# alibaba/TorchEasyRec

Hardware: NVIDIA H100
Metric: samples/sec (DLRM-Criteo synth, train step fwd+bwd+optimizer) (higher is better)
Workload: dtype f32

## Files before the change

include/tzk.h:

```cpp
#ifndef TZK_H_
#define TZK_H_

#include <stddef.h>
#include <stdint.h>

#ifdef __cplusplus
extern "C" {
#endif

#define TZK_ABI_VERSION 1

#define TZK_POOL_SUM 0
#define TZK_POOL_MEAN 1

#define TZK_OPT_SGD 0
#define TZK_OPT_ADAGRAD 1
#define TZK_OPT_ROWWISE_ADAGRAD 2
#define TZK_OPT_ADAM 3
#define TZK_OPT_PARTIAL_ROWWISE_ADAM 4
#define TZK_OPT_LAMB 5
#define TZK_OPT_PARTIAL_ROWWISE_LAMB 6
#define TZK_OPT_LARS_SGD 7
#define TZK_OPT_ACCUM_OUT 100

// ... 53 lines not shown
                                   const int64_t* offsets, const float* per_sample_weights, int32_t F, int32_t B,
                                   int32_t max_dim, int32_t vec_ok, float* out, int64_t ld_out, tzk_stream_t stream);

size_t tzk_fused_bwd_workspace_bytes(int64_t nnz, int64_t total_keys, int32_t max_dim);
int tzk_fused_bwd(int32_t optimizer, int32_t pooled, const float* grad_out, int64_t ld_grad,
                  const int64_t* feat_w_off, const int64_t* feat_rows, const int32_t* feat_dim,
                  const int32_t* feat_col, const int32_t* feat_pool, const int64_t* feat_key_base,
                  const int64_t* ids, const int64_t* offsets, int32_t F, int32_t B, int64_t nnz,
                  int64_t total_keys, int32_t max_dim, int32_t vec_ok, float* weights, float* state,
                  float lr, float eps, float grad_scale, void* workspace, size_t workspace_bytes,
                  tzk_stream_t stream);
int tzk_fused_bwd_ex(const tzk_opt_args* opt, int32_t pooled, const float* grad_out, int64_t ld_grad,
                     const int64_t* feat_w_off, const int64_t* feat_rows, const int32_t* feat_dim,
                     const int32_t* feat_col, const int32_t* feat_pool, const int64_t* feat_key_base,
                     const int64_t* ids, const int64_t* offsets, int32_t F, int32_t B, int64_t nnz,
                     int64_t total_keys, int32_t max_dim, int32_t vec_ok, float* weights, float grad_scale,
                     void* workspace, size_t workspace_bytes, tzk_stream_t stream);
int tzk_fused_bwd_apply_ex(const tzk_opt_args* opt, int32_t pooled, const float* grad_out, int64_t ld_grad,
                           const int64_t* feat_w_off, const int64_t* feat_rows, const int32_t* feat_dim,
                           const int32_t* feat_col, const int32_t* feat_pool, const int64_t* feat_key_base,
                           const int64_t* offsets, int32_t F, int32_t B, int64_t nnz, int64_t total_keys,
                           int32_t max_dim, int32_t vec_ok, float* weights, float grad_scale, void* workspace,
                           size_t workspace_bytes, tzk_stream_t stream);
int tzk_fused_bwd_sort(int32_t pooled, const int64_t* feat_rows, const int64_t* feat_key_base, const int64_t* ids,
                       const int64_t* offsets, int32_t F, int32_t B, int64_t nnz, int64_t total_keys,
                       int32_t max_dim, void* workspace, size_t workspace_bytes, tzk_stream_t stream);
int tzk_fused_bwd_apply(int32_t optimizer, int32_t pooled, const float* grad_out, int64_t ld_grad,
                        const int64_t* feat_w_off, const int64_t* feat_rows, const int32_t* feat_dim,
                        const int32_t* feat_col, const int32_t* feat_pool, const int64_t* feat_key_base,
                        const int64_t* offsets, int32_t F, int32_t B, int64_t nnz, int64_t total_keys,
                        int32_t max_dim, int32_t vec_ok, float* weights, float* state, float lr, float eps,
                        float grad_scale, void* workspace, size_t workspace_bytes, tzk_stream_t stream);

size_t tzk_fused_bwd_weighted_workspace_bytes(int64_t nnz, int64_t total_keys, int32_t max_dim);
int tzk_fused_bwd_sort_weighted(int32_t pooled, const int64_t* feat_rows, const int64_t* feat_key_base, const int64_t* ids,
                                const int64_t* offsets, const float* per_sample_weights, int32_t F, int32_t B,
                                int64_t nnz, int64_t total_keys, int32_t max_dim, void* workspace,
                                size_t workspace_bytes, tzk_stream_t stream);

int tzk_bag_grad_expand(const float* grad_out, int64_t ld_grad, const int32_t* feat_col,
                        const int32_t* feat_pool, const int64_t* offsets, const int32_t* slot, int32_t F,
                        int32_t B, int32_t D, float* g_rows, tzk_stream_t stream);

size_t tzk_bucketize_rw_workspace_bytes(int32_t F, int32_t B, int32_t W, int64_t nnz);
int tzk_bucketize_rw(const int64_t* ids, const int64_t* offsets, int32_t F, int32_t B, int32_t W,
                     const int64_t* feat_block, const int32_t* feat_owner, int64_t nnz,
                     int64_t wire_capacity, int32_t* out_lengths, int64_t* out_offsets, int64_t* out_ids,
                     int32_t* out_pos, int32_t* out_inv, void* workspace, size_t workspace_bytes,
                     tzk_stream_t stream);

int tzk_permute_lengths(const int32_t* lengths, const int32_t* perm, int32_t S_out, int32_t B,
                        int32_t* out_lengths, tzk_stream_t stream);
int tzk_permute_ids(const int64_t* ids, const int64_t* in_offsets, const int64_t* out_offsets,
                    const int32_t* perm, int32_t S_out, int32_t B, int64_t* out_ids,
                    tzk_stream_t stream);
int tzk_permute_weights(const float* weights, const int64_t* in_offsets, const int64_t* out_offsets,
                        const int32_t* perm, int32_t S_out, int32_t B, float* out_weights, tzk_stream_t stream);

int tzk_col_gather_sum(const float* const* srcs_host, const int64_t* src_ld_host, int32_t n_src,
                       const int32_t* col_start, const int32_t* col_src, const int32_t* col_srccol,
                       int32_t C, int64_t rows, float* out, int64_t ld_out, tzk_stream_t stream);

int tzk_jagged_to_padded(const float* values, const int64_t* offsets, int32_t B, int32_t T, int32_t D,
                         float* out, tzk_stream_t stream);
int tzk_padded_to_jagged(const float* grad_out, const int64_t* offsets, int32_t B, int32_t T, int32_t D,
                         int64_t nnz, float* grad_values, tzk_stream_t stream);

int tzk_fm_fwd(const float* x, int64_t ld_x, int64_t B, int32_t N, int32_t D, float* y, int64_t ld_y,
               tzk_stream_t stream);
int tzk_fm_bwd(const float* x, int64_t ld_x, const float* dy, int64_t ld_dy, int64_t B, int32_t N,
               int32_t D, float* dx, int64_t ld_dx, tzk_stream_t stream);

int tzk_dot_interact_fwd(const float* dense, int64_t ld_dense, const float* sparse, int64_t ld_sparse,
                         int64_t B, int32_t Ns, int32_t D, int32_t copy_dense, int32_t copy_sparse,
                         int32_t p_pad, float* out, int64_t ld_out, tzk_stream_t stream);
int tzk_dot_interact_bwd(const float* dense, int64_t ld_dense, const float* sparse, int64_t ld_sparse,
                         const float* d_out, int64_t ld_dout, int64_t B, int32_t Ns, int32_t D,
                         int32_t copy_dense, int32_t copy_sparse, int32_t p_pad, float* d_dense,
                         int64_t ld_ddense, float* d_sparse, int64_t ld_dsparse, tzk_stream_t stream);
int tzk_interact_wide_bwd(const float* dz, int64_t ld_dz, const float* w, int64_t ld_w, const float* dense,
                          int64_t ld_dense, const float* sparse, int64_t ld_sparse, int64_t M, float* d_dense,
                          int64_t ld_ddense, float* d_sparse, int64_t ld_dsparse, float* wt_hi, float* wt_lo,
                          tzk_stream_t stream);
int tzk_interact_wide_fwd(const float* dense, int64_t ld_dense, const float* sparse, int64_t ld_sparse, const float* w,
                          int64_t ld_w, const float* bias, int64_t M, float* y, int64_t ld_y, float* pairs,
                          int64_t ld_pairs, float* w_hi, float* w_lo, tzk_stream_t stream);
int tzk_interact_wide_wgrad(const float* dz, int64_t ld_dz, const float* pairs, int64_t ld_pairs, const float* dense,
                            int64_t ld_dense, const float* sparse, int64_t ld_sparse, int64_t M, int32_t slabs,
                            float* partial, float* dw, int64_t ld_dw, tzk_stream_t stream);

int tzk_bias_act(float* y, int64_t ld_y, const float* bias, int64_t M, int32_t N, int32_t relu,
                 tzk_stream_t stream);
size_t tzk_act_bwd_colsum_workspace_bytes(int64_t M, int32_t N);
int tzk_act_bwd_colsum(const float* dy, int64_t ld_dy, const float* y, int64_t ld_y, int64_t M, int32_t N,
                       int32_t relu, float* dz, int64_t ld_dz, float* colsum, void* workspace,
                       size_t workspace_bytes, tzk_stream_t stream);

int tzk_small_linear_fwd(const float* x, int64_t ld_x, const float* w, const float* bias, int64_t M, int32_t K,
                         int32_t N, int32_t relu, float* y, int64_t ld_y, tzk_stream_t stream);
size_t tzk_small_linear_bwd_workspace_bytes(int64_t M, int32_t K, int32_t N);
int tzk_small_linear_bwd(const float* x, int64_t ld_x, const float* w, const float* y, int64_t ld_y,
                         const float* dy, int64_t ld_dy, int64_t M, int32_t K, int32_t N, int32_t relu, float* dx,
                         int64_t ld_dx, float* dw, float* db, void* workspace, size_t workspace_bytes,
                         tzk_stream_t stream);
size_t tzk_bce_logits_workspace_bytes(int64_t M);

size_t tzk_tower_tail_bce_workspace_bytes(int64_t M, int32_t K, int32_t N);
int tzk_tower_tail_bce(const float* y1, int64_t ld_y, const float* w1, const float* b1, const float* w2, const float* b2,
                       const float* labels, int64_t M, int32_t K, int32_t N, float* logits, float* dy1, int64_t ld_dy,
                       float* out, void* workspace, size_t workspace_bytes, tzk_stream_t stream);
int tzk_bce_logits_fwd_bwd(const float* logits, const float* labels, int64_t M, float* loss, float* dlogits,
                           void* workspace, size_t workspace_bytes, tzk_stream_t stream);

int tzk_din_attn_input_fwd(const float* query, int64_t ld_q, int32_t Dq, const float* seq, const int64_t* offsets,
                           int32_t B, int32_t Ds, int64_t N, float* out, tzk_stream_t stream);
int tzk_din_attn_input_bwd(const float* d_in, const float* query, int64_t ld_q, int32_t Dq, const float* seq,
                           const int64_t* offsets, int32_t B, int32_t Ds, int64_t N, float* d_query, float* d_seq,
                           tzk_stream_t stream);
int tzk_jagged_softmax_wsum_fwd(const float* scores, const float* seq, const int64_t* offsets, int32_t B, int32_t Ds,
                                int32_t max_len, int64_t N, float* probs, float* out, tzk_stream_t stream);
int tzk_jagged_softmax_wsum_bwd(const float* d_out, const float* probs, const float* seq, const int64_t* offsets,
                                int32_t B, int32_t Ds, int32_t max_len, int64_t N, float* d_scores, float* d_seq,
                                tzk_stream_t stream);

int tzk_peer_pooled_gather_fwd(const uint64_t* table_ptrs, const int64_t* rf_w_off, const int64_t* feat_rows,
                               const int64_t* feat_block, const int32_t* feat_owner, const int32_t* feat_dim,
                               const int32_t* feat_col, const int32_t* feat_pool, const int64_t* ids,
                               const int64_t* offsets, int32_t F, int32_t B, int32_t W, int32_t max_dim, float* out,
                               int64_t ld_out, const float* mirror, const int64_t* feat_mirror_off, tzk_stream_t stream);
int tzk_peer_pooled_gather_fwd_sel(const uint64_t* table_ptrs, const int64_t* rf_w_off, const int64_t* feat_rows,
                                   const int64_t* feat_block, const int32_t* feat_owner, const int32_t* feat_dim,
                                   const int32_t* feat_col, const int32_t* feat_pool, const int64_t* ids,
                                   const int64_t* offsets, int32_t F, int32_t B, int32_t W, int32_t max_dim, float* out,
                                   int64_t ld_out, const float* mirror, const int64_t* feat_mirror_off,
                                   const int32_t* feat_sel, int32_t n_sel, tzk_stream_t stream);
int tzk_peer_seq_gather_fwd(const uint64_t* table_ptrs, const int64_t* rf_w_off, const int64_t* feat_rows,
                            const int64_t* feat_block, const int32_t* feat_owner, const int64_t* ids,
                            const int64_t* offsets, int32_t F, int32_t B, int32_t W, int32_t D, int64_t nnz, float* out,
                            const float* mirror, const int64_t* feat_mirror_off, tzk_stream_t stream);
int tzk_peer_mirror_refresh(const uint64_t* table_ptrs, int32_t W, const int32_t* seg_rank, const int64_t* seg_src,
                            const int64_t* seg_dst, const int64_t* seg_n, int32_t n_seg, float* mirror,
                            tzk_stream_t stream);
int tzk_peer_barrier(const uint64_t* pad_ptrs, int32_t me, int32_t W, uint32_t* epoch, tzk_stream_t stream);
size_t tzk_peer_bucketize_workspace_bytes(int32_t F, int32_t B, int32_t W);
int tzk_peer_bucketize(const int64_t* ids, const int64_t* offsets, int32_t F, int32_t B, int32_t W,
                       const int64_t* feat_block, const int32_t* feat_owner, const int64_t* feat_rows,
                       const int64_t* rf_key_base, int32_t pooled, int64_t cap, int64_t* wire_key, int32_t* wire_idx,
                       int32_t* counts, void* workspace, size_t workspace_bytes, tzk_stream_t stream);
int tzk_peer_publish_grad(const float* grad, int64_t ld_grad, const int32_t* feat_col, const int32_t* feat_dim,
                          const int32_t* feat_pool, const int64_t* offsets, int32_t F, int32_t B, float* dst,
                          int64_t ld_dst, tzk_stream_t stream);
int tzk_peer_push_grad(const uint64_t* recv_ptrs, const float* grad, int64_t ld_grad, const int32_t* feat_col,
                       const int32_t* feat_pool, const int64_t* offsets, const int32_t* wire_idx, const int32_t* counts,
                       int32_t me, int32_t W, int64_t cap, int32_t B, int32_t D, int32_t pooled, tzk_stream_t stream);
int tzk_peer_allreduce_mean(const uint64_t* src_ptrs, int32_t W, int64_t n, float* out, tzk_stream_t stream);
int tzk_peer_small_update(const tzk_opt_args* opt, const uint64_t* psum_ptrs, const uint64_t* flag_ptrs, int32_t W,
                          const void* tabs, int32_t n_tabs, int32_t total_rows, int32_t max_dim, float* weights,
                          tzk_stream_t stream);
int tzk_fused_bwd_sort_peer(const uint64_t* key_ptrs, const uint64_t* idx_ptrs, const uint64_t* count_ptrs, int32_t me,
                            int32_t W, int64_t cap, int32_t idx_span, int64_t total_keys, int32_t max_dim,
                            int32_t* overflow, void* workspace, size_t workspace_bytes, tzk_stream_t stream);
int tzk_fused_bwd_apply_peer(const tzk_opt_args* opt, int32_t pooled, const uint64_t* grad_ptrs, int64_t ld_grad,
                             const int64_t* feat_w_off, const int64_t* feat_rows, const int32_t* feat_dim,
                             const int32_t* feat_col, const int32_t* feat_pool, const int64_t* feat_key_base, int32_t F,
                             int32_t B, int32_t me, int32_t W, int64_t cap, int32_t idx_span, int64_t total_keys,
                             int32_t max_dim, int32_t vec_ok, float* weights, float grad_scale, void* workspace,
                             size_t workspace_bytes, tzk_stream_t stream);

int tzk_peer_pooled_gather_fwd_weighted(const uint64_t* table_ptrs, const int64_t* rf_w_off, const int64_t* feat_rows,
                                        const int64_t* feat_block, const int32_t* feat_owner, const int32_t* feat_dim,
                                        const int32_t* feat_col, const int32_t* feat_pool, const int64_t* ids,
                                        const int64_t* offsets, int32_t F, int32_t B, int32_t W, int32_t max_dim,
                                        float* out, int64_t ld_out, const float* mirror, const int64_t* feat_mirror_off,
                                        const float* per_sample_weights, const int32_t* feat_sel, int32_t n_sel,
                                        tzk_stream_t stream);
int tzk_peer_bucketize_weighted(const int64_t* ids, const int64_t* offsets, int32_t F, int32_t B, int32_t W,
                                const int64_t* feat_block, const int32_t* feat_owner, const int64_t* feat_rows,
                                const int64_t* rf_key_base, int32_t pooled, int64_t cap, int64_t* wire_key,
                                int32_t* wire_idx, int32_t* counts, void* workspace, size_t workspace_bytes,
                                const float* per_sample_weights, float* wire_w, tzk_stream_t stream);
int tzk_peer_push_grad_weighted(const uint64_t* recv_ptrs, const float* grad, int64_t ld_grad, const int32_t* feat_col,
                                const int32_t* feat_pool, const int64_t* offsets, const int32_t* wire_idx,
                                const int32_t* counts, int32_t me, int32_t W, int64_t cap, int32_t B, int32_t D,
                                int32_t pooled, const float* wire_w, tzk_stream_t stream);

int tzk_dot_interact27_fwd_bf16(const uint16_t* dense, int64_t ld_dense, const float* sparse, int64_t ld_sparse, int64_t B,
                                uint16_t* out, int64_t ld_out, tzk_stream_t stream);
int tzk_dot_interact27_bwd_bf16(const uint16_t* d_out, int64_t ld_dout, const uint16_t* dense, int64_t ld_dense,
                                const float* sparse, int64_t ld_sparse, int64_t B, uint16_t* d_dense, int64_t ld_ddense,
                                float* d_sparse, int64_t ld_dsparse, tzk_stream_t stream);

int tzk_binned_auc_update(const void* preds, int32_t pred_dtype, const void* labels, int32_t label_dtype, int64_t n,
                          const float* thresholds, int32_t T, int64_t* counts, int64_t* invalid, tzk_stream_t stream);
// ... 145 lines not shown
```

torcheasyrec_b200/_lib.py:

```python

import ctypes
import os
from ctypes import c_char_p, c_float, c_int32, c_int64, c_size_t, c_void_p

_HERE = os.path.dirname(os.path.abspath(__file__))
LIB_PATH = os.path.join(_HERE, "csrc", "libtzk.so")

P = c_void_p

class TzkOptArgs(ctypes.Structure):

    _fields_ = [("optimizer", c_int32), ("lr", c_float), ("eps", c_float), ("beta1", c_float), ("beta2", c_float),
                ("weight_decay", c_float), ("max_gradient", c_float), ("state", c_void_p), ("state2", c_void_p),
                ("step", c_void_p), ("weights_f16", c_int32), ("interleaved", c_int32), ("momentum", c_float),
                ("eta", c_float), ("weight_decay_mode", c_int32), ("per_sample_weights", c_void_p)]


PLE_MAX_GATES, PLE_MAX_EXPERTS, PLE_MAX_GATE_EXPERTS = 9, 64, 32


class TzkPleGateArgs(ctypes.Structure):

    _fields_ = [("B", c_int64), ("H", c_int32), ("n_experts", c_int32), ("n_inputs", c_int32), ("n_gates", c_int32),
                ("in_dim", c_int32 * PLE_MAX_GATES), ("gate_input", c_int32 * PLE_MAX_GATES),
# ... 46 lines not shown
    "tzk_sm_count": (c_int32, []),
    "tzk_lengths_to_offsets_workspace_bytes": (c_size_t, [c_int64]),
    "tzk_lengths_to_offsets": (c_int32, [P, c_int64, P, P, c_size_t, P]),
    "tzk_pooled_gather_fwd": (
        c_int32,
        [P, P, P, P, P, P, P, P, c_int32, c_int32, c_int32, c_int32, P, c_int64, P],
    ),
    "tzk_seq_gather_fwd": (c_int32, [P, P, P, P, P, c_int32, c_int32, c_int32, c_int64, P, P]),
    "tzk_pooled_gather_fwd_f16": (
        c_int32,
        [P, P, P, P, P, P, P, P, c_int32, c_int32, c_int32, c_int32, P, c_int64, P],
    ),
    "tzk_seq_gather_fwd_f16": (c_int32, [P, P, P, P, P, c_int32, c_int32, c_int32, c_int64, P, P]),
    "tzk_pooled_gather_fwd_strided": (
        c_int32,
        [P, P, P, P, P, P, P, P, P, c_int32, c_int32, c_int32, c_int32, P, c_int64, P],
    ),
    "tzk_seq_gather_fwd_strided": (c_int32, [P, P, P, P, P, c_int32, c_int32, c_int32, c_int32, c_int64, P, P]),
    "tzk_pooled_gather_fwd_weighted": (
        c_int32,
        [P, c_int32, P, P, P, P, P, P, P, P, P, c_int32, c_int32, c_int32, c_int32, P, c_int64, P],
    ),
    "tzk_fused_bwd_workspace_bytes": (c_size_t, [c_int64, c_int64, c_int32]),
    "tzk_fused_bwd_weighted_workspace_bytes": (c_size_t, [c_int64, c_int64, c_int32]),
    "tzk_fused_bwd_sort_weighted": (
        c_int32, [c_int32, P, P, P, P, P, c_int32, c_int32, c_int64, c_int64, c_int32, P, c_size_t, P]),
    "tzk_fused_bwd": (
        c_int32,
        [c_int32, c_int32, P, c_int64, P, P, P, P, P, P, P, P, c_int32, c_int32, c_int64, c_int64, c_int32,
         c_int32, P, P, c_float, c_float, c_float, P, c_size_t, P],
    ),
    "tzk_fused_bwd_ex": (
        c_int32,
        [P, c_int32, P, c_int64, P, P, P, P, P, P, P, P, c_int32, c_int32, c_int64, c_int64, c_int32, c_int32, P,
         c_float, P, c_size_t, P],
    ),
    "tzk_fused_bwd_apply_ex": (
        c_int32,
        [P, c_int32, P, c_int64, P, P, P, P, P, P, P, c_int32, c_int32, c_int64, c_int64, c_int32, c_int32, P,
         c_float, P, c_size_t, P],
    ),
    "tzk_fused_bwd_sort": (c_int32, [c_int32, P, P, P, P, c_int32, c_int32, c_int64, c_int64, c_int32, P, c_size_t, P]),
    "tzk_fused_bwd_apply": (
        c_int32,
        [c_int32, c_int32, P, c_int64, P, P, P, P, P, P, P, c_int32, c_int32, c_int64, c_int64, c_int32,
         c_int32, P, P, c_float, c_float, c_float, P, c_size_t, P],
    ),
    "tzk_bucketize_rw_workspace_bytes": (c_size_t, [c_int32, c_int32, c_int32, c_int64]),
    "tzk_bucketize_rw": (
        c_int32,
        [P, P, c_int32, c_int32, c_int32, P, P, c_int64, c_int64, P, P, P, P, P, P, c_size_t, P],
    ),
    "tzk_bag_grad_expand": (c_int32, [P, c_int64, P, P, P, P, c_int32, c_int32, c_int32, P, P]),
    "tzk_permute_lengths": (c_int32, [P, P, c_int32, c_int32, P, P]),
    "tzk_permute_ids": (c_int32, [P, P, P, P, c_int32, c_int32, P, P]),
    "tzk_permute_weights": (c_int32, [P, P, P, P, c_int32, c_int32, P, P]),
    "tzk_col_gather_sum": (c_int32, [P, P, c_int32, P, P, P, c_int32, c_int64, P, c_int64, P]),
    "tzk_jagged_to_padded": (c_int32, [P, P, c_int32, c_int32, c_int32, P, P]),
    "tzk_padded_to_jagged": (c_int32, [P, P, c_int32, c_int32, c_int32, c_int64, P, P]),
    "tzk_fm_fwd": (c_int32, [P, c_int64, c_int64, c_int32, c_int32, P, c_int64, P]),
    "tzk_fm_bwd": (c_int32, [P, c_int64, P, c_int64, c_int64, c_int32, c_int32, P, c_int64, P]),
    "tzk_dot_interact_fwd": (
        c_int32,
        [P, c_int64, P, c_int64, c_int64, c_int32, c_int32, c_int32, c_int32, c_int32, P, c_int64, P],
    ),
    "tzk_bias_act": (c_int32, [P, c_int64, P, c_int64, c_int32, c_int32, P]),
    "tzk_act_bwd_colsum_workspace_bytes": (c_size_t, [c_int64, c_int32]),
    "tzk_act_bwd_colsum": (c_int32, [P, c_int64, P, c_int64, c_int64, c_int32, c_int32, P, c_int64, P, P, c_size_t, P]),
    "tzk_small_linear_fwd": (c_int32, [P, c_int64, P, P, c_int64, c_int32, c_int32, c_int32, P, c_int64, P]),
    "tzk_small_linear_bwd_workspace_bytes": (c_size_t, [c_int64, c_int32, c_int32]),
    "tzk_small_linear_bwd": (
        c_int32,
        [P, c_int64, P, P, c_int64, P, c_int64, c_int64, c_int32, c_int32, c_int32, P, c_int64, P, P, P, c_size_t, P],
    ),
    "tzk_bce_logits_workspace_bytes": (c_size_t, [c_int64]),
    "tzk_bce_logits_fwd_bwd": (c_int32, [P, P, c_int64, P, P, P, c_size_t, P]),
    "tzk_dot_interact_bwd": (
        c_int32,
        [P, c_int64, P, c_int64, P, c_int64, c_int64, c_int32, c_int32, c_int32, c_int32, c_int32, P, c_int64, P,
         c_int64, P],
    ),
    "tzk_interact_wide_bwd": (
        c_int32, [P, c_int64, P, c_int64, P, c_int64, P, c_int64, c_int64, P, c_int64, P, c_int64, P, P, P]),
    "tzk_interact_wide_fwd": (
        c_int32, [P, c_int64, P, c_int64, P, c_int64, P, c_int64, P, c_int64, P, c_int64, P, P, P]),
    "tzk_interact_wide_wgrad": (
        c_int32, [P, c_int64, P, c_int64, P, c_int64, P, c_int64, c_int64, c_int32, P, P, c_int64, P]),
    "tzk_tower_tail_bce_workspace_bytes": (c_size_t, [c_int64, c_int32, c_int32]),
    "tzk_tower_tail_bce": (c_int32, [P, c_int64, P, P, P, P, P, c_int64, c_int32, c_int32, P, P, c_int64, P, P, c_size_t, P]),
    "tzk_din_attn_input_fwd": (c_int32, [P, c_int64, c_int32, P, P, c_int32, c_int32, c_int64, P, P]),
    "tzk_din_attn_input_bwd": (c_int32, [P, P, c_int64, c_int32, P, P, c_int32, c_int32, c_int64, P, P, P]),
    "tzk_jagged_softmax_wsum_fwd": (c_int32, [P, P, P, c_int32, c_int32, c_int32, c_int64, P, P, P]),
    "tzk_jagged_softmax_wsum_bwd": (c_int32, [P, P, P, P, c_int32, c_int32, c_int32, c_int64, P, P, P]),
    "tzk_peer_pooled_gather_fwd": (
        c_int32, [P, P, P, P, P, P, P, P, P, P, c_int32, c_int32, c_int32, c_int32, P, c_int64, P, P, P]),
    "tzk_peer_pooled_gather_fwd_sel": (
        c_int32, [P, P, P, P, P, P, P, P, P, P, c_int32, c_int32, c_int32, c_int32, P, c_int64, P, P, P, c_int32, P]),
    "tzk_peer_seq_gather_fwd": (
        c_int32, [P, P, P, P, P, P, P, c_int32, c_int32, c_int32, c_int32, c_int64, P, P, P, P]),
    "tzk_peer_mirror_refresh": (c_int32, [P, c_int32, P, P, P, P, c_int32, P, P]),
    "tzk_peer_barrier": (c_int32, [P, c_int32, c_int32, P, P]),
    "tzk_peer_bucketize_workspace_bytes": (c_size_t, [c_int32, c_int32, c_int32]),
    "tzk_peer_bucketize": (
        c_int32, [P, P, c_int32, c_int32, c_int32, P, P, P, P, c_int32, c_int64, P, P, P, P, c_size_t, P]),
    "tzk_peer_publish_grad": (c_int32, [P, c_int64, P, P, P, P, c_int32, c_int32, P, c_int64, P]),
    "tzk_peer_push_grad": (
        c_int32, [P, P, c_int64, P, P, P, P, P, c_int32, c_int32, c_int64, c_int32, c_int32, c_int32, P]),
    "tzk_peer_allreduce_mean": (c_int32, [P, c_int32, c_int64, P, P]),
    "tzk_peer_small_update": (c_int32, [P, P, P, c_int32, P, c_int32, c_int32, c_int32, P, P]),
    "tzk_fused_bwd_sort_peer": (
        c_int32, [P, P, P, c_int32, c_int32, c_int64, c_int32, c_int64, c_int32, P, P, c_size_t, P]),
    "tzk_fused_bwd_apply_peer": (
        c_int32,
        [P, c_int32, P, c_int64, P, P, P, P, P, P, c_int32, c_int32, c_int32, c_int32, c_int64, c_int32, c_int64,
         c_int32, c_int32, P, c_float, P, c_size_t, P]),
    "tzk_peer_pooled_gather_fwd_weighted": (
        c_int32, [P, P, P, P, P, P, P, P, P, P, c_int32, c_int32, c_int32, c_int32, P, c_int64, P, P, P, P, c_int32, P]),
    "tzk_peer_bucketize_weighted": (
        c_int32, [P, P, c_int32, c_int32, c_int32, P, P, P, P, c_int32, c_int64, P, P, P, P, c_size_t, P, P, P]),
    "tzk_peer_push_grad_weighted": (
        c_int32, [P, P, c_int64, P, P, P, P, P, c_int32, c_int32, c_int64, c_int32, c_int32, c_int32, P, P]),
    "tzk_dot_interact27_fwd_bf16": (c_int32, [P, c_int64, P, c_int64, c_int64, P, c_int64, P]),
    "tzk_dot_interact27_bwd_bf16": (
        c_int32, [P, c_int64, P, c_int64, P, c_int64, c_int64, P, c_int64, P, c_int64, P]),
    "tzk_binned_auc_update": (c_int32, [P, c_int32, P, c_int32, c_int64, P, c_int32, P, P, P]),
    "tzk_peer_pooled_gather_fwd_f16": (
        c_int32, [P, P, P, P, P, P, P, P, P, P, c_int32, c_int32, c_int32, c_int32, P, c_int64, P, P, P]),
    "tzk_peer_pooled_gather_fwd_sel_f16": (
        c_int32, [P, P, P, P, P, P, P, P, P, P, c_int32, c_int32, c_int32, c_int32, P, c_int64, P, P, P, c_int32, P]),
    "tzk_peer_pooled_gather_fwd_weighted_f16": (
        c_int32, [P, P, P, P, P, P, P, P, P, P, c_int32, c_int32, c_int32, c_int32, P, c_int64, P, P, P, P, c_int32, P]),
    "tzk_peer_seq_gather_fwd_f16": (
        c_int32, [P, P, P, P, P, P, P, c_int32, c_int32, c_int32, c_int32, c_int64, P, P, P, P]),
    "tzk_peer_mirror_refresh_f16": (c_int32, [P, c_int32, P, P, P, P, c_int32, P, P]),
    "tzk_wukong_mix_fwd": (
        c_int32, [P, P, P, P, P, P, c_int64, c_int32, c_int32, c_int32, c_int32, c_int32, c_int32, P, P, P, P]),
    "tzk_wukong_mix_bwd": (
        c_int32,
        [P, P, P, P, P, P, P, P, c_int64, c_int32, c_int32, c_int32, c_int32, c_int32, c_int32, P, P, P, P]),
    "tzk_wukong_out_fwd": (c_int32, [P, P, P, P, c_int64, c_int32, c_int32, c_int32, c_int32, P, P, P]),
    "tzk_wukong_out_bwd": (
        c_int32, [P, P, P, P, P, c_int64, c_int32, c_int32, c_int32, c_int32, P, P, P, P, P]),
    "tzk_masknet_mask_fwd": (c_int32, [P, c_int32, P, P, P, P, c_int64, c_int32, c_int32, c_int32, P, P, P]),
    "tzk_masknet_mask_bwd": (
        c_int32, [P, c_int32, P, P, P, P, P, P, c_int64, c_int32, c_int32, c_int32, P, P, P, P, P]),
    "tzk_masknet_ffn_fwd": (c_int32, [P, P, P, P, c_int64, c_int32, c_int32, c_int32, P, P, P]),
    "tzk_masknet_ffn_bwd": (c_int32, [P, P, P, P, P, P, c_int64, c_int32, c_int32, c_int32, P, P, P, P]),
    "tzk_ple_gate_smem_bytes": (c_int64, [P, c_int32]),
    "tzk_ple_gate_fwd": (c_int32, [P, c_int32, P, P, P]),
    "tzk_ple_gate_bwd": (c_int32, [P, P, P, c_int32, P, P, P, P]),
    "tzk_pepnet_gate_fwd": (c_int32, [P, c_int32, P]),
    "tzk_pepnet_gate_bwd": (c_int32, [P, c_int32, P, P, P]),
    "tzk_jrc_loss_workspace_bytes": (c_size_t, [c_int64]),
    "tzk_jrc_loss": (c_int32, [P, c_int64, P, P, P, c_int64, c_float, c_int32, P, P, P, c_size_t, P]),
    "tzk_rocket_head_fwd": (c_int32, [P, c_int32, P, P, P]),
    "tzk_rocket_head_bwd": (c_int32, [P, P, P, c_int32, P, P, P]),
}

_lib = None


class TzkError(RuntimeError):
    pass


def lib() -> ctypes.CDLL:
    global _lib
    if _lib is None:
        if not os.path.exists(LIB_PATH):
            raise TzkError(
                f"{LIB_PATH} not found: build it with `python -m torcheasyrec_b200.csrc.build` "
                "(or __graft_entry__.build()).  There is no CPU fallback."
# ... 17 lines not shown
```

torcheasyrec_b200/csrc/tzk_common.cuh:

```cuda
#pragma once
#include <stdlib.h>
#include <cuda_fp16.h>
#include <cuda_runtime.h>
#include <stdint.h>
#include <stdio.h>

#include "../../include/tzk.h"

namespace tzk {

void set_error(const char* fmt, ...);

inline cudaStream_t as_stream(tzk_stream_t s) { return reinterpret_cast<cudaStream_t>(s); }

#define TZK_CHECK_LAUNCH(name)                                                      \
  do {                                                                              \
    cudaError_t e__ = cudaGetLastError();                                           \
    if (e__ != cudaSuccess) {                                                       \
      ::tzk::set_error("%s: launch failed: %s", name, cudaGetErrorString(e__));     \
      return 2;                                                                     \
    }                                                                               \
  } while (0)

#define TZK_REQUIRE(cond, ...)        \
  do {                                \
    if (!(cond)) {                    \
      ::tzk::set_error(__VA_ARGS__);  \
      return 1;                       \
    }                                 \
  } while (0)

constexpr int kSmCountH100 = 132;

inline bool unvalidated_switch(const char* name) {
  const char* e = getenv(name);
  if (e && (e[0] == '0' || e[0] == '1')) return e[0] == '1';
  const char* x = getenv("TZK_EXPERIMENTAL");
  return x && x[0] == '1';
}

__host__ __device__ inline int64_t ceil_div64(int64_t a, int64_t b) { return (a + b - 1) / b; }
inline size_t align_up(size_t x, size_t a) { return (x + a - 1) / a * a; }
__host__ __device__ inline size_t align16(size_t x) { return (x + 15) / 16 * 16; }

__device__ __forceinline__ float4 ld_row_f4(const float* p) {
  float4 r;
  asm("ld.global.nc.L1::no_allocate.v4.f32 {%0,%1,%2,%3}, [%4];"
               : "=f"(r.x), "=f"(r.y), "=f"(r.z), "=f"(r.w)
               : "l"(p));
  return r;
}
__device__ __forceinline__ float4 ld_coh_f4(const float* p) {
  float4 r;
  asm("ld.global.L1::no_allocate.v4.f32 {%0,%1,%2,%3}, [%4];" : "=f"(r.x), "=f"(r.y), "=f"(r.z), "=f"(r.w) : "l"(p));
  return r;
}
__device__ __forceinline__ float4 ld_rw_f4(const float* p) {
  float4 r;
  asm volatile("ld.global.L1::no_allocate.v4.f32 {%0,%1,%2,%3}, [%4];"
               : "=f"(r.x), "=f"(r.y), "=f"(r.z), "=f"(r.w)
               : "l"(p)
               : "memory");
  return r;
}
__device__ __forceinline__ float4 ld_row_h4(const __half* p) {
  unsigned int a, b;
  asm("ld.global.nc.L1::no_allocate.v2.u32 {%0,%1}, [%2];" : "=r"(a), "=r"(b) : "l"(p));
  const float2 lo = __half22float2(*reinterpret_cast<const __half2*>(&a));
  const float2 hi = __half22float2(*reinterpret_cast<const __half2*>(&b));
  return make_float4(lo.x, lo.y, hi.x, hi.y);
}
template <typename WT> __device__ __forceinline__ float4 ld_table_f4(const WT* p);
template <> __device__ __forceinline__ float4 ld_table_f4<float>(const float* p) { return ld_row_f4(p); }
template <> __device__ __forceinline__ float4 ld_table_f4<__half>(const __half* p) { return ld_row_h4(p); }
template <typename WT> __device__ __forceinline__ float ld_table_f1(const WT* p);
template <> __device__ __forceinline__ float ld_table_f1<float>(const float* p) { return __ldg(p); }
template <> __device__ __forceinline__ float ld_table_f1<__half>(const __half* p) { return __half2float(__ldg(p)); }

__device__ __forceinline__ void st_stream_f4(float* p, const float4& v) {
  asm volatile("st.global.L1::no_allocate.v4.f32 [%0], {%1,%2,%3,%4};" ::"l"(p), "f"(v.x), "f"(v.y),
               "f"(v.z), "f"(v.w)
               : "memory");
}
__device__ __forceinline__ float4 f4_add(const float4& a, const float4& b) {
  return make_float4(a.x + b.x, a.y + b.y, a.z + b.z, a.w + b.w);
}
__device__ __forceinline__ float4 f4_scale(const float4& a, float s) {
  return make_float4(a.x * s, a.y * s, a.z * s, a.w * s);
}

}
```

torcheasyrec_b200/csrc/tzk_dense.cu:

```cuda
#include <cstdlib>

#include "tzk_common.cuh"

using namespace tzk;

#include "tzk_launch.cuh"
namespace tzk_itc {
__device__ __forceinline__ uint32_t cvt_tf32(float x) {
  uint32_t r;
  asm("cvt.rna.tf32.f32 %0, %1;" : "=r"(r) : "f"(x));
  return r;
}
__device__ __forceinline__ void mma_tf32(float (&c)[4], const uint32_t (&a)[4], const uint32_t (&b)[2]) {
  asm volatile("mma.sync.aligned.m16n8k8.row.col.f32.tf32.tf32.f32 {%0,%1,%2,%3}, {%4,%5,%6,%7}, {%8,%9}, {%0,%1,%2,%3};"
               : "+f"(c[0]), "+f"(c[1]), "+f"(c[2]), "+f"(c[3])
               : "r"(a[0]), "r"(a[1]), "r"(a[2]), "r"(a[3]), "r"(b[0]), "r"(b[1]));
}
}
#include "tzk_interact_tc.cuh"


namespace {
constexpr int kThreads = 256;

// ... 657 lines not shown
  const int64_t stride = (int64_t)gridDim.x * blockDim.x;
  for (int64_t i = (int64_t)blockIdx.x * blockDim.x + threadIdx.x; i < n; i += stride) {
    const int64_t r = i / N;
    const int c = (int)(i - r * N);
    float v = y[r * ld + c] + (bias ? __ldg(bias + c) : 0.f);
    if (relu) v = v > 0.f ? v : 0.f;
    y[r * ld + c] = v;
  }
}

__global__ void __launch_bounds__(kThreads)
bias_act_vec_kernel(float* __restrict__ y, int64_t ld, const float* __restrict__ bias, int n4_total, int N4,
                    int relu) {
  const int stride = gridDim.x * blockDim.x;
  for (int i = blockIdx.x * blockDim.x + threadIdx.x; i < n4_total; i += stride) {
    const int r = i / N4, c4 = i - r * N4;
    float4* p = reinterpret_cast<float4*>(y + (int64_t)r * ld) + c4;
    float4 v = *p;
    if (bias) {
      const float4 b = __ldg(reinterpret_cast<const float4*>(bias) + c4);
      v.x += b.x; v.y += b.y; v.z += b.z; v.w += b.w;
    }
    if (relu) {
      v.x = v.x > 0.f ? v.x : 0.f; v.y = v.y > 0.f ? v.y : 0.f;
      v.z = v.z > 0.f ? v.z : 0.f; v.w = v.w > 0.f ? v.w : 0.f;
    }
    *p = v;
  }
}

constexpr int kSlabRows = 128;
__global__ void __launch_bounds__(kThreads)
act_bwd_colsum_kernel(const float* __restrict__ dy, int64_t ld_dy, const float* __restrict__ y, int64_t ld_y,
                      int64_t M, int N, int relu, float* __restrict__ dz, int64_t ld_dz,
                      float* __restrict__ partial) {
  __shared__ float red[kThreads];
  const int rg = kThreads / N;
  const int c = threadIdx.x % N, r0 = threadIdx.x / N;
  const int64_t row_lo = (int64_t)blockIdx.x * kSlabRows;
  const int64_t row_hi = row_lo + kSlabRows < M ? row_lo + kSlabRows : M;
  float acc = 0.f;
#pragma unroll 4
  for (int64_t r = row_lo + r0; r < row_hi; r += rg) {
    float g = __ldg(dy + r * ld_dy + c);
    if (relu && !(__ldg(y + r * ld_y + c) > 0.f)) g = 0.f;
    if (dz) dz[r * ld_dz + c] = g;
    acc += g;
  }
  red[threadIdx.x] = acc;
  __syncthreads();
  if (r0 == 0) {
    float s = 0.f;
    for (int k = 0; k < rg; ++k) s += red[k * N + c];
    partial[(int64_t)blockIdx.x * N + c] = s;
  }
}

__global__ void __launch_bounds__(256)
colsum_final_kernel(const float* __restrict__ partial, int64_t n_blocks, int N, float* __restrict__ out) {
  __shared__ float red[8][32];
  const int o = threadIdx.x & 31, g = threadIdx.x >> 5;
  const int c = blockIdx.x * 32 + o;
  float s = 0.f;
  if (c < N) {
    int64_t b = g;
    for (; b + 24 < n_blocks; b += 32) {
      const float a0 = partial[b * N + c], a1 = partial[(b + 8) * N + c];
      const float a2 = partial[(b + 16) * N + c], a3 = partial[(b + 24) * N + c];
      s += a0; s += a1; s += a2; s += a3;
    }
    for (; b < n_blocks; b += 8) s += partial[b * N + c];
  }
  red[g][o] = s;
  __syncthreads();
  if (g == 0 && c < N) {
    float r = 0.f;
#pragma unroll
    for (int k = 0; k < 8; ++k) r += red[k][o];
    out[c] = r;
  }
}
}

extern "C" int tzk_bias_act(float* y, int64_t ld_y, const float* bias, int64_t M, int32_t N, int32_t relu,
                            tzk_stream_t stream) {
  TZK_REQUIRE(M >= 0 && N >= 1, "bias_act: bad sizes");
  if (M == 0) return 0;
  TZK_REQUIRE(y != nullptr, "bias_act: y is NULL");
  const bool vec = (N % 4 == 0) && (ld_y % 4 == 0) && ((uintptr_t)y % 16 == 0) &&
                   (!bias || (uintptr_t)bias % 16 == 0) && (M * N / 4 < ((int64_t)1 << 31));
  if (vec)
    bias_act_vec_kernel<<<grid_for(M * N / 4, kThreads, kSmCountH100 * 16), kThreads, 0, as_stream(stream)>>>(
        y, ld_y, bias, (int)(M * N / 4), N / 4, relu);
  else
    bias_act_kernel<<<grid_for(M * N, kThreads, kSmCountH100 * 16), kThreads, 0, as_stream(stream)>>>(y, ld_y, bias,
                                                                                                    M, N, relu);
  TZK_CHECK_LAUNCH("bias_act_kernel");
  return 0;
}

extern "C" size_t tzk_act_bwd_colsum_workspace_bytes(int64_t M, int32_t N) {
  return (size_t)ceil_div64(M < 1 ? 1 : M, kSlabRows) * (size_t)(N < 1 ? 1 : N) * sizeof(float);
}

extern "C" int tzk_act_bwd_colsum(const float* dy, int64_t ld_dy, const float* y, int64_t ld_y, int64_t M,
                                  int32_t N, int32_t relu, float* dz, int64_t ld_dz, float* colsum,
                                  void* workspace, size_t workspace_bytes, tzk_stream_t stream) {
  TZK_REQUIRE(M >= 1 && N >= 1, "act_bwd_colsum: bad sizes");
  TZK_REQUIRE(N <= kThreads && kThreads % N == 0, "act_bwd_colsum: N=%d must divide %d", N, kThreads);
  TZK_REQUIRE(dy && colsum && (!relu || y), "act_bwd_colsum: NULL argument");
  TZK_REQUIRE(workspace && workspace_bytes >= tzk_act_bwd_colsum_workspace_bytes(M, N),
              "act_bwd_colsum: workspace too small");
  const int64_t nb = ceil_div64(M, kSlabRows);
  float* partial = static_cast<float*>(workspace);
  act_bwd_colsum_kernel<<<(unsigned)nb, kThreads, 0, as_stream(stream)>>>(dy, ld_dy, y, ld_y, M, N, relu, dz, ld_dz,
                                                                          partial);
  TZK_CHECK_LAUNCH("act_bwd_colsum_kernel");
  colsum_final_kernel<<<(N + 31) / 32, 256, 0, as_stream(stream)>>>(partial, nb, N, colsum);
  TZK_CHECK_LAUNCH("colsum_final_kernel");
  return 0;
}
```

torcheasyrec_b200/csrc/tzk_interact_wide.cu:

```cuda
#include <stdint.h>
#include <stdio.h>
#include <stdlib.h>

#ifdef TZK_CPU_SHIM
#include "cuda_cpu_shim.h"
#include "sm90_cpu_emu.h"
#include "sm90_wgmma_emu.h"
typedef void* tzk_stream_t;
inline void mbar_arrive(uint64_t* bar) { mbar_expect_tx(bar, 0); }
#define TZK_REQUIRE(cond, ...) do { if (!(cond)) return 1; } while (0)
#define TZK_CHECK_LAUNCH(name) do {} while (0)
#else
#include <cuda.h>
#include "tzk_common.cuh"
#define TZK_DYN_SMEM(type, name) extern __shared__ __align__(1024) type name[]
#include "tzk_launch.cuh"
#endif

namespace {
#ifndef TZK_CPU_SHIM
#include "tzk_sm90_ptx.h"
#endif
#include "tzk_tma.h"
#include "tzk_wgmma.cuh"
namespace tzk_itc {
__device__ __forceinline__ uint32_t cvt_tf32(float x) { return tf32_bits(x); }
__device__ __forceinline__ void mma_tf32(float (&c)[4], const uint32_t (&a)[4], const uint32_t (&b)[2]) { ::mma_tf32(c, a, b); }
}
#include "tzk_interact_tc.cuh"

__device__ __forceinline__ float4 load_l2(const float* p) {
#ifdef TZK_CPU_SHIM
  return *reinterpret_cast<const float4*>(p);
#else
  return __ldcg(reinterpret_cast<const float4*>(p));
#endif
}

constexpr int FB_M = 64;
constexpr int FB_THREADS = 512;
constexpr int FB_WARPS = FB_THREADS / 32;
constexpr int FB_CHUNKS = (tzk_itc::kRow + 31) / 32;
constexpr int FB_PAIR_CHUNKS = tzk_itc::kInter / 32;
constexpr int FB_ITEMS = 1 + FB_CHUNKS;
constexpr int FB_BOX = 32 * 128;
constexpr int FB_HALF = 2 * FB_BOX;
constexpr int FB_STAGE = 2 * FB_HALF;
constexpr int FB_STAGES = 4;
constexpr int FB_LDP = 360;
constexpr int FB_P_OFF = FB_STAGES * FB_STAGE;
constexpr int FB_S_OFF = FB_P_OFF + FB_M * FB_LDP * 4;
constexpr int FB_IJ_OFF = FB_S_OFF + FB_WARPS * 32 * tzk_itc::kSS * 4;
constexpr int FB_BAR_OFF = FB_IJ_OFF + tzk_itc::kInter * 2;
constexpr int FB_SMEM = FB_BAR_OFF + 4 * FB_STAGES * 8;
static_assert(FB_HALF == FB_M * 128, "a dZ box [64 x 32 floats] fills half a stage");
static_assert(FB_STAGES == 4, "stage i % 4 is read by warpgroup i % 4");
static_assert(FB_SMEM <= 227 * 1024, "over the opt-in shared memory of one CTA");

#ifdef TZK_FB_TIMING
__device__ unsigned long long* fb_timing;
__device__ __forceinline__ unsigned long long fb_now() {
  unsigned long long t;
  asm volatile("mov.u64 %0, %%globaltimer;" : "=l"(t));
  return t;
}
#define FB_STAMP(tile, slot) do { if (threadIdx.x == 0) fb_timing[4 * (tile) + (slot)] = fb_now(); } while (0)
#define FB_STAMP_LAST(tile, slot) do { if ((threadIdx.x & 31) == 0) atomicMax(fb_timing + 4 * (tile) + (slot), fb_now()); } while (0)
#else
#define FB_STAMP(tile, slot) do {} while (0)
#define FB_STAMP_LAST(tile, slot) do {} while (0)
#endif

struct FbParams {
  const float* dense; int64_t ld_dense;
  const float* sparse; int64_t ld_sparse;
  float* d_dense; int64_t ld_ddense;
  float* d_sparse; int64_t ld_dsparse;
  int64_t M;
};

__global__ void __launch_bounds__(FB_THREADS, 1)
interact_wide_bwd_kernel(const __grid_constant__ CUtensorMap map_dz, const __grid_constant__ CUtensorMap map_whi,
                         const __grid_constant__ CUtensorMap map_wlo, FbParams p) {
  TZK_DYN_SMEM(uint8_t, smem);
  float* P = reinterpret_cast<float*>(smem + FB_P_OFF);
  uint64_t* full = reinterpret_cast<uint64_t*>(smem + FB_BAR_OFF);
  uint64_t* empty = full + 2 * FB_STAGES;
  const int warp = threadIdx.x >> 5, lane = threadIdx.x & 31, g = lane >> 2, t = lane & 3;
  const int wg = warp >> 2, r = (warp & 3) * 16 + g;
  const int64_t tiles = (p.M + FB_M - 1) / FB_M;

  if (threadIdx.x == 0) {
    for (int s = 0; s < 2 * FB_STAGES; ++s) {
      mbar_init(full + s, 1);
      mbar_init(empty + s, 4);
    }
    fence_mbarrier_init();
  }
  float* S = reinterpret_cast<float*>(smem + FB_S_OFF) + warp * (32 * tzk_itc::kSS);
  unsigned short* pair_ij = reinterpret_cast<unsigned short*>(smem + FB_IJ_OFF);
  tzk_itc::init_pair_ij(pair_ij);
  for (int i = lane; i < 32 * tzk_itc::kSS; i += 32) S[i] = 0.f;
  __syncthreads();
  auto load = [&](int64_t item, int h) {
    const int64_t tile = blockIdx.x + item / FB_ITEMS * gridDim.x;
    if (tile >= tiles) return;
    if (item >= FB_STAGES) mbar_wait(empty + 2 * (item % FB_STAGES) + h, (uint32_t)(item / FB_STAGES - 1) & 1u);
    const int j = (int)(item % FB_ITEMS);
    uint8_t* hb = smem + (item % FB_STAGES) * FB_STAGE + h * FB_HALF;
    uint64_t* bar = full + 2 * (item % FB_STAGES) + h;
    mbar_expect_tx(bar, FB_HALF);
    if (j == 0) {
      tma_load_2d(hb, &map_dz, bar, 32 * h, (int)(tile * FB_M));
    } else {
      tma_load_2d(hb, &map_whi, bar, 32 * h, (j - 1) * 32);
      tma_load_2d(hb + FB_BOX, &map_wlo, bar, 32 * h, (j - 1) * 32);
    }
  };
  if (threadIdx.x == 0)
    for (int i = 0; i < FB_STAGES; ++i) {
      load(i, 0);
      load(i, 1);
    }

  int64_t item0 = 0;
  for (int64_t tile = blockIdx.x; tile < tiles; tile += gridDim.x, item0 += FB_ITEMS) {
    const int64_t m0 = tile * FB_M;
    FB_STAMP(tile, 0);
    float a[8][4];
    {
      const int s = (int)(item0 % FB_STAGES);
      mbar_wait(full + 2 * s, (uint32_t)(item0 / FB_STAGES) & 1u);
      mbar_wait(full + 2 * s + 1, (uint32_t)(item0 / FB_STAGES) & 1u);
      const float* zs = reinterpret_cast<const float*>(smem + s * FB_STAGE);
#pragma unroll
      for (int kk = 0; kk < 8; ++kk) {
        const float* box = zs + (kk >> 2) * (FB_HALF / 4);
        const int k0 = (kk & 3) * 8 + t, k1 = k0 + 4;
        a[kk][0] = box[swz(r, k0)];
        a[kk][1] = box[swz(r + 8, k0)];
        a[kk][2] = box[swz(r, k1)];
        a[kk][3] = box[swz(r + 8, k1)];
      }
    }
    __syncthreads();
    if (warp < 4 && lane == 0) {
      mbar_arrive(empty + 2 * (item0 % FB_STAGES));
      mbar_arrive(empty + 2 * (item0 % FB_STAGES) + 1);
    }
    if (threadIdx.x == 0) {
      load(item0 + FB_STAGES, 0);
      load(item0 + FB_STAGES, 1);
    }
    FB_STAMP(tile, 1);

    for (int c = (int)((wg - item0 - 1) & 3); c < FB_CHUNKS; c += 4) {
      const int64_t item = item0 + 1 + c;
      float acc[16], part[16];
#pragma unroll
      for (int i = 0; i < 16; ++i) acc[i] = 0.f;
#pragma unroll
      for (int kk = 0; kk < 8; ++kk) {
        const int h = kk >> 2;
        const uint8_t* whi = smem + wg * FB_STAGE + h * FB_HALF;
        if ((kk & 3) == 0) mbar_wait(full + 2 * wg + h, (uint32_t)(item / FB_STAGES) & 1u);
        uint32_t ah[4], al[4];
#pragma unroll
        for (int i = 0; i < 4; ++i) {
          ah[i] = tf32_bits(a[kk][i]);
          al[i] = tf32_bits(a[kk][i] - __uint_as_float(ah[i]));
        }
        wgmma_fence();
        wgmma_3xtf32<32>(part, ah, al, wgmma_desc(whi, kk & 3), wgmma_desc(whi + FB_BOX, kk & 3));
        wgmma_commit();
        wgmma_wait<0>();
#pragma unroll
        for (int i = 0; i < 16; ++i) {
          wgmma_reg_fence(part[i]);
          acc[i] += part[i];
        }
        if ((kk & 3) == 3) {
          __syncwarp();
          if (lane == 0) mbar_arrive(empty + 2 * wg + h);
          if ((threadIdx.x & 127) == 0) load(item + FB_STAGES, h);
        }
      }
#pragma unroll
      for (int i = 0; i < 4; ++i) {
        const int col = c * 32 + i * 8 + 2 * t;
        if (col < tzk_itc::kInter) {
          *reinterpret_cast<float2*>(P + r * FB_LDP + col) = make_float2(acc[4 * i], acc[4 * i + 1]);
          *reinterpret_cast<float2*>(P + (r + 8) * FB_LDP + col) = make_float2(acc[4 * i + 2], acc[4 * i + 3]);
        } else if (col < tzk_itc::kRow) {
          const int e = col - tzk_itc::kInter;
#pragma unroll
          for (int h = 0; h < 2; ++h) {
            const int64_t row = m0 + r + 8 * h;
            if (row >= p.M) continue;
            float* dst = e < tzk_itc::kD ? p.d_dense + row * p.ld_ddense + e : p.d_sparse + row * p.ld_dsparse + (e - tzk_itc::kD);
            *reinterpret_cast<float2*>(dst) = make_float2(acc[4 * i + 2 * h], acc[4 * i + 2 * h + 1]);
          }
        }
      }
    }
    __syncthreads();
    FB_STAMP(tile, 2);

    for (int i = warp; i < FB_M; i += FB_WARPS) {
      const int64_t b = m0 + i;
      if (b >= p.M) break;
      float* dd = p.d_dense + b * p.ld_ddense;
      float* ds = p.d_sparse + b * p.ld_dsparse;
      float4 pass[4];
#pragma unroll
      for (int q = 0; q < 4; ++q) {
        const int row = g + 8 * q;
        pass[q] = row == 0 ? load_l2(dd + 4 * t)
                : row < tzk_itc::kN ? load_l2(ds + (row - 1) * tzk_itc::kD + 4 * t)
                : make_float4(0.f, 0.f, 0.f, 0.f);
      }
      tzk_itc::bwd_sample(P + i * FB_LDP, p.dense + b * p.ld_dense, p.sparse + b * p.ld_sparse, pass, pair_ij, S, dd, ds,
                          lane);
    }
    FB_STAMP_LAST(tile, 3);
  }
// ... 130 lines not shown
    const float b0 = p.bias ? __ldg(p.bias + col) : 0.f, b1 = p.bias ? __ldg(p.bias + col + 1) : 0.f;
#pragma unroll
    for (int h = 0; h < 2; ++h) {
      const int64_t row = m0 + r + 8 * h;
      if (row >= p.M) continue;
      float2 o = make_float2(acc[4 * nt + 2 * h] + b0, acc[4 * nt + 2 * h + 1] + b1);
      o.x = fmaxf(o.x, 0.f);
      o.y = fmaxf(o.y, 0.f);
      *reinterpret_cast<float2*>(p.y + row * p.ld_y + col) = o;
    }
  }
}

__global__ void split_w_kernel(const float* __restrict__ w, int64_t ld_w, int K, float* __restrict__ hi,
                               float* __restrict__ lo) {
  const int i = blockIdx.x * blockDim.x + threadIdx.x;
  if (i < K * 64) {
    const float v = w[(int64_t)(i / K) * ld_w + i % K];
    const float h = tf32_rna(v);
    hi[i] = h;
    lo[i] = tf32_rna(v - h);
  }
}

#include "tzk_wgrad3x.cuh"

constexpr int WW_ZT = 64 * 128;

__global__ void __launch_bounds__(WG_THREADS, 2)
interact_wide_wgrad_kernel(const __grid_constant__ CUtensorMap map_x0, const __grid_constant__ CUtensorMap map_x1,
                           const __grid_constant__ CUtensorMap map_x2, const __grid_constant__ CUtensorMap map_dz,
                           WgParams p) {
  TZK_DYN_SMEM(uint8_t, smem);
  uint8_t* zt = smem + WG_STAGES * WG_STAGE;
  uint64_t* full = reinterpret_cast<uint64_t*>(zt + 2 * WW_ZT);
  int* boxes = reinterpret_cast<int*>(full + WG_STAGES);

  const int warp = threadIdx.x >> 5, lane = threadIdx.x & 31, g = lane >> 2, t = lane & 3;
  const int jt = blockIdx.x % p.k_tiles;
  const int64_t slab = blockIdx.x / p.k_tiles;
  const int64_t row0 = slab * p.slab_rows;
  const int64_t rows = (p.M - row0 < p.slab_rows) ? p.M - row0 : p.slab_rows;
  const int num_c = (int)((rows + WG_ROWS - 1) / WG_ROWS);

  if (threadIdx.x == 0) {
    for (int s = 0; s < WG_STAGES; ++s) mbar_init(full + s, 1);
    fence_mbarrier_init();
    for (int b = 0; b < 4; ++b) {
      const int box = jt * 4 + b, s = wg_source(p.src, box);
      boxes[b] = s;
      boxes[4 + b] = wg_pick(p.src.col0, s) + 32 * (box - wg_pick(p.src.first, s));
    }
  }
  __syncthreads();
  auto load = [&](int c) {
    uint8_t* sb = smem + (c % WG_STAGES) * WG_STAGE;
    uint64_t* bar = full + c % WG_STAGES;
    const int r = (int)(row0 + (int64_t)c * WG_ROWS);
    mbar_expect_tx(bar, WG_A + WG_B);
#pragma unroll 1
    for (int b = 0; b < 4; ++b) {
      const int s = *reinterpret_cast<volatile int*>(boxes + b), col = *reinterpret_cast<volatile int*>(boxes + 4 + b);
      tma_load_2d(sb + b * WG_BOX, s == 0 ? &map_x0 : s == 1 ? &map_x1 : &map_x2, bar, col, r);
    }
#pragma unroll
    for (int b = 0; b < 2; ++b) tma_load_2d(sb + WG_A + b * WG_BOX, &map_dz, bar, b * 32, r);
  };
  if (threadIdx.x == 0)
    for (int c = 0; c < WG_STAGES && c < num_c; ++c) load(c);

  const int xc = (warp >> 2) * 64 + (warp & 3) * 16 + g;
  const int tn = threadIdx.x & 63, tq = threadIdx.x >> 6;
  uint32_t* zhi = reinterpret_cast<uint32_t*>(zt);
  uint32_t* zlo = zhi + WW_ZT / 4;
  float acc[32], part[32];
#pragma unroll
  for (int i = 0; i < 32; ++i) acc[i] = 0.f;
  for (int c = 0; c < num_c; ++c) {
    const int s = c % WG_STAGES;
    mbar_wait(full + s, (uint32_t)(c / WG_STAGES) & 1u);
    const float* xs = reinterpret_cast<const float*>(smem + s * WG_STAGE);
    const float* zs = reinterpret_cast<const float*>(smem + s * WG_STAGE + WG_A);
    auto at = [](const float* base, int m, int col) { return base[(col >> 5) * (WG_BOX / 4) + swz(m, col & 31)]; };
#pragma unroll
    for (int h = 0; h < 2; ++h) {
      const int m = 4 * tq + 16 * h;
      float hi[4], lo[4];
#pragma unroll
      for (int j = 0; j < 4; ++j) {
        const float v = at(zs, m + j, tn);
        hi[j] = tf32_rna(v);
        lo[j] = tf32_rna(v - hi[j]);
      }
      *reinterpret_cast<float4*>(zhi + swz(tn, m)) = make_float4(hi[0], hi[1], hi[2], hi[3]);
      *reinterpret_cast<float4*>(zlo + swz(tn, m)) = make_float4(lo[0], lo[1], lo[2], lo[3]);
    }
    fence_proxy_async();
    __syncthreads();
#pragma unroll
    for (int ks = 0; ks < WG_ROWS / 8; ++ks) {
      const int m = ks * 8 + t;
      const float a[4] = {at(xs, m, xc), at(xs, m, xc + 8), at(xs, m + 4, xc), at(xs, m + 4, xc + 8)};
      uint32_t ah[4], al[4];
#pragma unroll
      for (int i = 0; i < 4; ++i) {
        ah[i] = tf32_bits(a[i]);
        al[i] = tf32_bits(a[i] - __uint_as_float(ah[i]));
      }
      wgmma_fence();
      wgmma_tf32<64>(part, ah, wgmma_desc(zlo, ks), false);
      wgmma_tf32<64>(part, al, wgmma_desc(zhi, ks), true);
      wgmma_tf32<64>(part, ah, wgmma_desc(zhi, ks), true);
      wgmma_commit();
      wgmma_wait<0>();
#pragma unroll
      for (int i = 0; i < 32; ++i) {
        wgmma_reg_fence(part[i]);
        acc[i] += part[i];
      }
    }
    __syncthreads();
    if (threadIdx.x == 0 && c + WG_STAGES < num_c) load(c + WG_STAGES);
  }
  float* out = p.partial + ((int64_t)slab * p.k_tiles + jt) * 128 * 64;
#pragma unroll
  for (int i = 0; i < 8; ++i)
#pragma unroll
    for (int h = 0; h < 2; ++h)
      *reinterpret_cast<float2*>(out + (int64_t)(xc + 8 * h) * 64 + 8 * i + 2 * t) =
          make_float2(acc[4 * i + 2 * h], acc[4 * i + 2 * h + 1]);
}

__global__ void split_wt_kernel(const float* __restrict__ w, int64_t ld_w, int K, float* __restrict__ hi,
                                float* __restrict__ lo) {
  const int i = blockIdx.x * blockDim.x + threadIdx.x;
  if (i < K * 64) {
    const int k = i >> 6, o = i & 63;
    const float v = w[(int64_t)o * ld_w + k];
    const float h = tf32_rna(v);
    hi[i] = h;
    lo[i] = tf32_rna(v - h);
  }
}

}

#ifdef TZK_FB_TIMING
extern "C" int tzk_interact_wide_bwd_timing(unsigned long long* buf) {
  return cudaMemcpyToSymbol(fb_timing, &buf, sizeof(buf)) == cudaSuccess ? 0 : 1;
}
#endif

extern "C" int tzk_interact_wide_bwd(const float* dz, int64_t ld_dz, const float* w, int64_t ld_w, const float* dense,
                                     int64_t ld_dense, const float* sparse, int64_t ld_sparse, int64_t M, float* d_dense,
                                     int64_t ld_ddense, float* d_sparse, int64_t ld_dsparse, float* wt_hi, float* wt_lo,
                                     tzk_stream_t stream) {
  TZK_REQUIRE(M > 0, "interact_wide_bwd: M must be positive");
  TZK_REQUIRE(ld_w >= tzk_itc::kRow, "interact_wide_bwd: w needs %d columns", tzk_itc::kRow);
  const int64_t lds[] = {ld_dz, ld_w, ld_dense, ld_sparse, ld_ddense, ld_dsparse};
  for (int64_t ld : lds) TZK_REQUIRE(ld % 4 == 0, "interact_wide_bwd: row strides must be multiples of 4 floats");
  const void* ptrs[] = {dz, w, dense, sparse, d_dense, d_sparse, wt_hi, wt_lo};
  for (const void* q : ptrs)
    TZK_REQUIRE(q && reinterpret_cast<uintptr_t>(q) % 16 == 0, "interact_wide_bwd: NULL or not 16-B aligned pointer");
  int dev = 0, sms = 0;
  TZK_REQUIRE(cudaGetDevice(&dev) == cudaSuccess &&
              cudaDeviceGetAttribute(&sms, cudaDevAttrMultiProcessorCount, dev) == cudaSuccess && sms > 0,
              "interact_wide_bwd: no device");
#ifdef TZK_CPU_SHIM
  if (const char* e = getenv("TZK_EMU_SMS")) sms = atoi(e);
#endif
  cudaStream_t st = reinterpret_cast<cudaStream_t>(stream);
  TZK_LAUNCH((split_wt_kernel), (tzk_itc::kRow * 64 + 255) / 256, 256, 0, st, w, ld_w, tzk_itc::kRow, wt_hi, wt_lo);
  CUtensorMap mz, mh, ml;
  TZK_REQUIRE(!make_map(&mz, dz, M, 64, ld_dz, FB_M) && !make_map(&mh, wt_hi, tzk_itc::kRow, 64, 64, 32) &&
              !make_map(&ml, wt_lo, tzk_itc::kRow, 64, 64, 32), "interact_wide_bwd: tensor-map encoding failed");
  FbParams p;
  p.dense = dense; p.ld_dense = ld_dense; p.sparse = sparse; p.ld_sparse = ld_sparse;
  p.d_dense = d_dense; p.ld_ddense = ld_ddense; p.d_sparse = d_sparse; p.ld_dsparse = ld_dsparse; p.M = M;
#ifndef TZK_CPU_SHIM
  static bool configured = false;
  if (!configured) {
    cudaFuncSetAttribute(interact_wide_bwd_kernel, cudaFuncAttributeMaxDynamicSharedMemorySize, FB_SMEM);
    configured = true;
  }
#endif
  const int64_t tiles = (M + FB_M - 1) / FB_M;
  TZK_LAUNCH((interact_wide_bwd_kernel), (unsigned)(tiles < sms ? tiles : sms), FB_THREADS, FB_SMEM, st, mz, mh, ml, p);
  TZK_CHECK_LAUNCH("interact_wide_bwd_kernel");
  return 0;
}

extern "C" int tzk_interact_wide_fwd(const float* dense, int64_t ld_dense, const float* sparse, int64_t ld_sparse,
                                     const float* w, int64_t ld_w, const float* bias, int64_t M, float* y, int64_t ld_y,
                                     float* pairs, int64_t ld_pairs, float* w_hi, float* w_lo, tzk_stream_t stream) {
  TZK_REQUIRE(M > 0, "interact_wide_fwd: M must be positive");
  TZK_REQUIRE(ld_w >= tzk_itc::kRow && ld_y >= 64 && ld_pairs >= tzk_itc::kInter && ld_dense >= tzk_itc::kD &&
              ld_sparse >= tzk_itc::kRow - FF_SPARSE0, "interact_wide_fwd: row stride shorter than the row");
  const int64_t lds[] = {ld_dense, ld_sparse, ld_w, ld_y, ld_pairs};
  for (int64_t ld : lds) TZK_REQUIRE(ld % 4 == 0, "interact_wide_fwd: row strides must be multiples of 4 floats");
  const void* ptrs[] = {dense, sparse, w, y, pairs, w_hi, w_lo};
  for (const void* q : ptrs)
    TZK_REQUIRE(q && reinterpret_cast<uintptr_t>(q) % 16 == 0, "interact_wide_fwd: NULL or not 16-B aligned pointer");
  cudaStream_t st = reinterpret_cast<cudaStream_t>(stream);
  TZK_LAUNCH((split_w_kernel), (tzk_itc::kRow * 64 + 255) / 256, 256, 0, st, w, ld_w, tzk_itc::kRow, w_hi, w_lo);
  CUtensorMap mp, md, ms, mh, ml;
  TZK_REQUIRE(!make_map(&mp, pairs, M, tzk_itc::kInter, ld_pairs, FF_M) &&
              !make_map(&md, dense, M, tzk_itc::kD, ld_dense, FF_M) &&
              !make_map(&ms, sparse, M, tzk_itc::kRow - FF_SPARSE0, ld_sparse, FF_M) &&
              !make_map(&mh, w_hi, 64, tzk_itc::kRow, tzk_itc::kRow, 64) &&
              !make_map(&ml, w_lo, 64, tzk_itc::kRow, tzk_itc::kRow, 64), "interact_wide_fwd: tensor-map encoding failed");
  FfParams p;
  p.dense = dense; p.ld_dense = ld_dense; p.sparse = sparse; p.ld_sparse = ld_sparse; p.pairs = pairs;
  p.ld_pairs = ld_pairs; p.bias = bias; p.y = y; p.ld_y = ld_y; p.M = M;
#ifndef TZK_CPU_SHIM
  static bool configured = false;
  if (!configured) {
    cudaFuncSetAttribute(interact_wide_fwd_kernel, cudaFuncAttributeMaxDynamicSharedMemorySize, FF_SMEM);
    configured = true;
  }
#endif
  TZK_LAUNCH((interact_wide_fwd_kernel), (unsigned)((M + FF_M - 1) / FF_M), FF_THREADS, FF_SMEM, st, mp, md, ms, mh, ml, p);
  TZK_CHECK_LAUNCH("interact_wide_fwd_kernel");
  return 0;
}

extern "C" int tzk_interact_wide_wgrad(const float* dz, int64_t ld_dz, const float* pairs, int64_t ld_pairs,
                                       const float* dense, int64_t ld_dense, const float* sparse, int64_t ld_sparse,
                                       int64_t M, int32_t slabs, float* partial, float* dw, int64_t ld_dw,
                                       tzk_stream_t stream) {
  TZK_REQUIRE(M > 0 && slabs > 0, "interact_wide_wgrad: M and slabs must be positive");
  TZK_REQUIRE(ld_dw >= tzk_itc::kRow, "interact_wide_wgrad: dw needs %d columns", tzk_itc::kRow);
  const int64_t lds[] = {ld_dz, ld_pairs, ld_dense, ld_sparse};
  for (int64_t ld : lds) TZK_REQUIRE(ld % 4 == 0, "interact_wide_wgrad: row strides must be multiples of 4 floats");
  const void* ptrs[] = {dz, pairs, dense, sparse, partial, dw};
  for (const void* q : ptrs)
    TZK_REQUIRE(q && reinterpret_cast<uintptr_t>(q) % 16 == 0, "interact_wide_wgrad: NULL or not 16-B aligned pointer");
  CUtensorMap mx[WG_SRC], mz;
  TZK_REQUIRE(!make_map(&mx[0], pairs, M, tzk_itc::kInter, ld_pairs, WG_ROWS) &&
              !make_map(&mx[1], sparse, M, tzk_itc::kRow - FF_SPARSE0, ld_sparse, WG_ROWS) &&
              !make_map(&mx[2], dense, M, tzk_itc::kD, ld_dense, WG_ROWS) &&
              !make_map(&mz, dz, M, 64, ld_dz, WG_ROWS), "interact_wide_wgrad: tensor-map encoding failed");
  const WgSources src = {{0, FB_PAIR_CHUNKS, FB_CHUNKS - 1, FB_CHUNKS}, {0, 0, 0}, {0, FF_SPARSE0, tzk_itc::kInter},
                         {tzk_itc::kInter, tzk_itc::kRow - FF_SPARSE0, tzk_itc::kD}};
  TZK_REQUIRE(wgrad3x_launch<interact_wide_wgrad_kernel>(mx, mz, src, M, slabs, partial, dw, ld_dw,
                                                         reinterpret_cast<cudaStream_t>(stream), 2 * WW_ZT) == 0,
              "interact_wide_wgrad: launch failed");
  return 0;
}
```

torcheasyrec_b200/csrc/tzk_tower.cu:

```cuda
#include <cstdlib>

#include "tzk_common.cuh"

#include "tzk_launch.cuh"
#include "tzk_tower_bwd2.cuh"
#include "tzk_tower_tail.cuh"

using namespace tzk;

namespace {
constexpr int kTM = 128;

__device__ __forceinline__ int odd(int v) { return v | 1; }
constexpr int kNW = kTM / 32;
constexpr int kLU = 16;

__device__ __forceinline__ void load_tile(float* dst, int S, const float* __restrict__ src, int64_t ld,
                                          const float* __restrict__ mask, int64_t ld_m, int rows, int C) {
  const int warp = threadIdx.x >> 5, lane = threadIdx.x & 31;
  for (int r0 = warp; r0 < rows; r0 += kNW * kLU) {
    float v[kLU][2], m[kLU][2];
#pragma unroll
    for (int q = 0; q < kLU; ++q) {
      const int r = r0 + q * kNW;
// ... 334 lines not shown
  return v1 > v2 ? v1 : v2;
}

extern "C" int tzk_small_linear_bwd(const float* x, int64_t ld_x, const float* w, const float* y, int64_t ld_y,
                                    const float* dy, int64_t ld_dy, int64_t M, int32_t K, int32_t N, int32_t relu,
                                    float* dx, int64_t ld_dx, float* dw, float* db, void* workspace,
                                    size_t workspace_bytes, tzk_stream_t stream) {
  int rc = small_linear_check("small_linear_bwd", M, K, N);
  if (rc) return rc;
  TZK_REQUIRE(M >= 1, "small_linear_bwd: empty batch");
  TZK_REQUIRE(x && w && dy && dw && (!relu || y), "small_linear_bwd: NULL argument");
  TZK_REQUIRE(ld_x >= K && ld_dy >= N && (!relu || ld_y >= N) && (!dx || ld_dx >= K),
              "small_linear_bwd: leading dimension smaller than the row");
  TZK_REQUIRE(workspace && workspace_bytes >= tzk_small_linear_bwd_workspace_bytes(M, K, N),
              "small_linear_bwd: workspace too small");
  if (use_bwd2(K, N)) {
    rc = tzk_bwd2::run(x, ld_x, w, y, ld_y, dy, ld_dy, M, K, N, relu, dx, ld_dx, dw, db, workspace, workspace_bytes,
                       as_stream(stream));
    TZK_REQUIRE(rc == 0, "small_linear_bwd: tzk_bwd2::run failed with code %d", rc);
    return 0;
  }
  const int KP = pad_pow(K, 16), NP = pad_pow(N, 4);
  const int grid = bwd_grid(M);
  const size_t smem = ((size_t)N * KP + (size_t)kTM * (K | 1) + (size_t)kTM * (N | 1)) * sizeof(float);
  float* partial = static_cast<float*>(workspace);
  cudaStream_t st = as_stream(stream);
#define TZK_SLB(KP_, NP_)                                                                                          \
  do {                                                                                                             \
    if (smem > 48 * 1024)                                                                                          \
      cudaFuncSetAttribute(small_linear_bwd_kernel<KP_, NP_>, cudaFuncAttributeMaxDynamicSharedMemorySize,         \
                           (int)smem);                                                                             \
    small_linear_bwd_kernel<KP_, NP_><<<grid, kTM, smem, st>>>(x, ld_x, w, y, ld_y, dy, ld_dy, M, K, N, relu, dx,   \
                                                               ld_dx, partial);                                    \
  } while (0)
#define TZK_SLB_N(KP_)                      \
  switch (NP) {                             \
    case 4: TZK_SLB(KP_, 4); break;         \
    case 16: TZK_SLB(KP_, 16); break;       \
    case 32: TZK_SLB(KP_, 32); break;       \
    default: TZK_SLB(KP_, 64); break;       \
  }
  switch (KP) {
    case 16: TZK_SLB_N(16) break;
    case 32: TZK_SLB_N(32) break;
    default: TZK_SLB_N(64) break;
  }
#undef TZK_SLB_N
#undef TZK_SLB
  TZK_CHECK_LAUNCH("small_linear_bwd_kernel");
  const int total = N * K + N;
  small_linear_reduce_kernel<<<(total + 31) / 32, 256, 0, st>>>(partial, grid, N * K, N, dw, db);
  TZK_CHECK_LAUNCH("small_linear_reduce_kernel");
  return 0;
}

extern "C" size_t tzk_bce_logits_workspace_bytes(int64_t M) {
  return (size_t)ceil_div64(M < 1 ? 1 : M, kBceThreads * kBcePerThread) * sizeof(float);
}

extern "C" int tzk_bce_logits_fwd_bwd(const float* logits, const float* labels, int64_t M, float* loss,
                                      float* dlogits, void* workspace, size_t workspace_bytes,
                                      tzk_stream_t stream) {
  TZK_REQUIRE(M >= 1, "bce_logits: empty batch");
  TZK_REQUIRE(logits && labels && loss, "bce_logits: NULL argument");
  TZK_REQUIRE(workspace && workspace_bytes >= tzk_bce_logits_workspace_bytes(M), "bce_logits: workspace too small");
  const int64_t nb = ceil_div64(M, kBceThreads * kBcePerThread);
  TZK_REQUIRE(nb < ((int64_t)1 << 31), "bce_logits: batch too large");
  float* partial = static_cast<float*>(workspace);
  cudaStream_t st = as_stream(stream);
  const float inv_m = 1.0f / (float)M;
  bce_fwd_bwd_kernel<<<(unsigned)nb, kBceThreads, 0, st>>>(logits, labels, M, inv_m, dlogits, partial);
  TZK_CHECK_LAUNCH("bce_fwd_bwd_kernel");
  bce_final_kernel<<<1, 256, 0, st>>>(partial, (int)nb, inv_m, loss);
  TZK_CHECK_LAUNCH("bce_final_kernel");
  return 0;
}

extern "C" size_t tzk_tower_tail_bce_workspace_bytes(int64_t M, int32_t K, int32_t N) {
  return tzk_tail::supported(K, N) ? tzk_tail::workspace_bytes(M < 1 ? 1 : M, K, N) : 0;
}

extern "C" int tzk_tower_tail_bce(const float* y1, int64_t ld_y, const float* w1, const float* b1, const float* w2,
                                  const float* b2, const float* labels, int64_t M, int32_t K, int32_t N, float* logits,
                                  float* dy1, int64_t ld_dy, float* out, void* workspace, size_t workspace_bytes,
                                  tzk_stream_t stream) {
  TZK_REQUIRE(M >= 1, "tower_tail_bce: empty batch");
  TZK_REQUIRE(tzk_tail::supported(K, N), "tower_tail_bce: K=%d, N=%d must be in [1, 64]", K, N);
  TZK_REQUIRE(y1 && w1 && w2 && labels && logits && dy1 && out, "tower_tail_bce: NULL argument");
  TZK_REQUIRE(ld_y >= K && ld_dy >= K, "tower_tail_bce: leading dimension smaller than the row");
  TZK_REQUIRE(workspace && workspace_bytes >= tzk_tower_tail_bce_workspace_bytes(M, K, N),
              "tower_tail_bce: workspace too small");
  const int rc = tzk_tail::run(y1, ld_y, w1, b1, w2, b2, labels, M, K, N, logits, dy1, ld_dy, out, workspace,
                               workspace_bytes, as_stream(stream));
  TZK_REQUIRE(rc == 0, "tower_tail_bce: tzk_tail::run failed with code %d", rc);
  return 0;
}
```

torcheasyrec_b200/csrc/tzk_tower_tail.cuh:

```cuda
#pragma once
#include <stdint.h>

namespace tzk_tail {
constexpr int kRows = 128;
constexpr int kMaxCtas = 132 * 4;

__device__ __forceinline__ bool aligned16(const void* p) { return (reinterpret_cast<uintptr_t>(p) & 15) == 0; }

inline int out_len(int K, int N) { return N * K + 2 * N + 2; }
inline int grid_for(int64_t M) {
  const int64_t t = (M + kRows - 1) / kRows;
  return (int)(t < 1 ? 1 : (t < kMaxCtas ? t : kMaxCtas));
}
inline size_t workspace_bytes(int64_t M, int K, int N) { return (size_t)grid_for(M) * out_len(K, N) * sizeof(float); }
inline size_t smem_bytes(int KP, int NP) {
  return ((size_t)NP * KP + 2 * NP + (size_t)kRows * (KP + 4) + 2 * (size_t)kRows * NP + 2 * kRows) * sizeof(float);
}

template <int KP, int NP>
__global__ void __launch_bounds__(kRows)
tower_tail_bce_kernel(const float* __restrict__ y1, int64_t ld_y, const float* __restrict__ w1,
                      const float* __restrict__ b1, const float* __restrict__ w2, const float* __restrict__ b2,
                      const float* __restrict__ labels, int64_t M, int K, int N, float inv_m, int rows_per_cta,
                      float* __restrict__ logits, float* __restrict__ dy1, int64_t ld_dy, float* __restrict__ partial) {
  constexpr int R = kRows, KC = KP / 4, NC = NP / 4, XS = KP + 4;
  constexpr int NB = (KC * NC + R - 1) / R;
  TZK_DYN_SMEM(float, sm);
  float* Ws = sm;
  float* b1s = Ws + NP * KP;
  float* w2s = b1s + NP;
  float* Xs = w2s + NP;
  float* Dh = Xs + R * XS;
  float* Hg = Dh + R * NP;
  float* Dz = Hg + R * NP;
  float* Ls = Dz + R;
  const int tid = threadIdx.x;
  for (int i = tid; i < NP * KP; i += R) {
    const int n = i / KP, k = i - n * KP;
    Ws[i] = (n < N && k < K) ? __ldg(w1 + (int64_t)n * K + k) : 0.f;
  }
  for (int n = tid; n < NP; n += R) {
    b1s[n] = (n < N && b1) ? __ldg(b1 + n) : 0.f;
    w2s[n] = n < N ? __ldg(w2 + n) : 0.f;
  }
  const float b2v = b2 ? __ldg(b2) : 0.f;
  const bool vin = (K & 3) == 0 && (ld_y & 3) == 0 && aligned16(y1);
  const bool vout = (K & 3) == 0 && (ld_dy & 3) == 0 && aligned16(dy1);
  float acc[NB][4][4], accv = 0.f, accw = 0.f, accz = 0.f, accl = 0.f;
#pragma unroll
  for (int q = 0; q < NB; ++q)
#pragma unroll
    for (int i = 0; i < 4; ++i)
#pragma unroll
      for (int j = 0; j < 4; ++j) acc[q][i][j] = 0.f;
  const int64_t row_begin = (int64_t)blockIdx.x * rows_per_cta;
  const int64_t row_end = row_begin + rows_per_cta < M ? row_begin + rows_per_cta : M;
  __syncthreads();
  for (int64_t t0 = row_begin; t0 < row_end; t0 += R) {
    const int64_t row = t0 + tid;
    const bool live = row < row_end;
    float* xr = Xs + tid * XS;
#pragma unroll
    for (int c = 0; c < KC; ++c) {
      float4 v = make_float4(0.f, 0.f, 0.f, 0.f);
      if (live && 4 * c < K) {
        const float* p = y1 + row * ld_y + 4 * c;
        if (vin) {
          v = *reinterpret_cast<const float4*>(p);
        } else {
          v.x = __ldg(p);
          if (4 * c + 1 < K) v.y = __ldg(p + 1);
          if (4 * c + 2 < K) v.z = __ldg(p + 2);
          if (4 * c + 3 < K) v.w = __ldg(p + 3);
        }
      }
      *reinterpret_cast<float4*>(xr + 4 * c) = v;
    }
    float h[NP];
#pragma unroll
    for (int n = 0; n < NP; ++n) h[n] = b1s[n];
#pragma unroll 2
    for (int c = 0; c < KC; ++c) {
      const float4 x4 = *reinterpret_cast<const float4*>(xr + 4 * c);
#pragma unroll
      for (int n = 0; n < NP; ++n) {
        const float4 w4 = *reinterpret_cast<const float4*>(Ws + n * KP + 4 * c);
        h[n] = fmaf(x4.x, w4.x, h[n]);
        h[n] = fmaf(x4.y, w4.y, h[n]);
        h[n] = fmaf(x4.z, w4.z, h[n]);
        h[n] = fmaf(x4.w, w4.w, h[n]);
      }
    }
    float z = b2v;
#pragma unroll
    for (int n = 0; n < NP; ++n) {
      h[n] = h[n] > 0.f ? h[n] : 0.f;
      z = fmaf(h[n], w2s[n], z);
    }
    float dz = 0.f, lt = 0.f;
    if (live) {
      const float y = __ldg(labels + row);
      const float e = expf(-fabsf(z));
      lt = fmaxf(z, 0.f) - z * y + log1pf(e);
      const float sig = z >= 0.f ? 1.f / (1.f + e) : e / (1.f + e);
      dz = (sig - y) * inv_m;
      logits[row] = z;
    }
    Dz[tid] = dz;
    Ls[tid] = lt;
#pragma unroll
    for (int n = 0; n < NP; ++n) {
      Hg[tid * NP + n] = dz * h[n];
      h[n] = h[n] > 0.f ? dz * w2s[n] : 0.f;
      Dh[tid * NP + n] = h[n];
    }
#pragma unroll 2
    for (int c = 0; c < KC; ++c) {
      float4 a = make_float4(0.f, 0.f, 0.f, 0.f);
#pragma unroll
      for (int n = 0; n < NP; ++n) {
        const float4 w4 = *reinterpret_cast<const float4*>(Ws + n * KP + 4 * c);
        a.x = fmaf(h[n], w4.x, a.x);
        a.y = fmaf(h[n], w4.y, a.y);
        a.z = fmaf(h[n], w4.z, a.z);
        a.w = fmaf(h[n], w4.w, a.w);
      }
      if (live && 4 * c < K) {
        float* p = dy1 + row * ld_dy + 4 * c;
        if (vout) {
          *reinterpret_cast<float4*>(p) = a;
        } else {
          p[0] = a.x;
          if (4 * c + 1 < K) p[1] = a.y;
          if (4 * c + 2 < K) p[2] = a.z;
          if (4 * c + 3 < K) p[3] = a.w;
        }
      }
    }
    __syncthreads();
#pragma unroll
    for (int q = 0; q < NB; ++q) {
      const int blk = tid + q * R;
      if (blk < KC * NC) {
        const int tn = blk / KC, tk = blk - tn * KC;
        const float* dp = Dh + 4 * tn;
        const float* xp = Xs + 4 * tk;
#pragma unroll 4
        for (int r = 0; r < R; ++r) {
          const float4 a4 = *reinterpret_cast<const float4*>(dp + r * NP);
          const float4 b4 = *reinterpret_cast<const float4*>(xp + r * XS);
          const float a[4] = {a4.x, a4.y, a4.z, a4.w}, b[4] = {b4.x, b4.y, b4.z, b4.w};
#pragma unroll
          for (int i = 0; i < 4; ++i)
#pragma unroll
            for (int j = 0; j < 4; ++j) acc[q][i][j] = fmaf(a[i], b[j], acc[q][i][j]);
        }
      }
    }
    if (tid < NP) {
      for (int r = 0; r < R; ++r) {
        accv += Dh[r * NP + tid];
        accw += Hg[r * NP + tid];
      }
    }
    if (tid == 0) {
      for (int r = 0; r < R; ++r) {
        accz += Dz[r];
        accl += Ls[r];
      }
    }
    __syncthreads();
  }
  float* out = partial + (int64_t)blockIdx.x * (N * K + 2 * N + 2);
#pragma unroll
  for (int q = 0; q < NB; ++q) {
    const int blk = tid + q * R;
    if (blk < KC * NC) {
      const int tn = blk / KC, tk = blk - tn * KC;
#pragma unroll
      for (int i = 0; i < 4; ++i)
#pragma unroll
        for (int j = 0; j < 4; ++j)
          if (4 * tn + i < N && 4 * tk + j < K) out[(4 * tn + i) * K + 4 * tk + j] = acc[q][i][j];
    }
  }
  if (tid < N) {
    out[N * K + tid] = accv;
    out[N * K + N + tid] = accw;
  }
  if (tid == 0) {
    out[N * K + 2 * N] = accz;
    out[N * K + 2 * N + 1] = accl;
  }
}

__global__ void __launch_bounds__(256)
tower_tail_reduce_kernel(const float* __restrict__ partial, int n_parts, int len, float inv_m, float* __restrict__ out) {
  __shared__ float red[8][32];
  const int o = threadIdx.x & 31, g = threadIdx.x >> 5;
  const int i = blockIdx.x * 32 + o;
  float s = 0.f;
  if (i < len)
    for (int c = g; c < n_parts; c += 8) s += partial[(int64_t)c * len + i];
  red[g][o] = s;
  __syncthreads();
  if (g == 0 && i < len) {
    float r = 0.f;
#pragma unroll
    for (int k = 0; k < 8; ++k) r += red[k][o];
    out[i] = i == len - 1 ? r * inv_m : r;
  }
}

inline bool supported(int K, int N) { return K >= 1 && N >= 1 && K <= 64 && N <= 64; }

inline int run(const float* y1, int64_t ld_y, const float* w1, const float* b1, const float* w2, const float* b2,
               const float* labels, int64_t M, int32_t K, int32_t N, float* logits, float* dy1, int64_t ld_dy,
               float* out, void* workspace, size_t workspace_bytes_, cudaStream_t st) {
  if (M < 1 || !supported(K, N) || !y1 || !w1 || !w2 || !labels || !logits || !dy1 || !out || ld_y < K || ld_dy < K) return 1;
  if (workspace_bytes_ < workspace_bytes(M, K, N)) return 2;
  const int KP = K <= 16 ? 16 : (K <= 32 ? 32 : 64);
  const int NP = N <= 16 ? 16 : (N <= 32 ? 32 : 64);
  const int grid = grid_for(M);
  int rows_per_cta = (int)((M + grid - 1) / grid);
  rows_per_cta = (rows_per_cta + kRows - 1) / kRows * kRows;
  const float inv_m = 1.0f / (float)M;
  const size_t smem = smem_bytes(KP, NP);
  float* partial = static_cast<float*>(workspace);
#ifdef TZK_CPU_SHIM
#define TZK_TAIL_ATTR(KP_, NP_)
#else
#define TZK_TAIL_ATTR(KP_, NP_)                                                                                       \
  if (smem > 48 * 1024)                                                                                               \
    cudaFuncSetAttribute(tower_tail_bce_kernel<KP_, NP_>, cudaFuncAttributeMaxDynamicSharedMemorySize, (int)smem);
#endif
#define TZK_TAIL(KP_, NP_)                                                                                            \
  do {                                                                                                                \
    TZK_TAIL_ATTR(KP_, NP_)                                                                                           \
    TZK_LAUNCH((tower_tail_bce_kernel<KP_, NP_>), grid, kRows, smem, st, y1, ld_y, w1, b1, w2, b2, labels, M, K, N,   \
               inv_m, rows_per_cta, logits, dy1, ld_dy, partial);                                                     \
  } while (0)
#define TZK_TAIL_N(KP_)                                                                                               \
  do {                                                                                                                \
    if (NP == 16) TZK_TAIL(KP_, 16);                                                                                  \
    else if (NP == 32) TZK_TAIL(KP_, 32);                                                                             \
    else TZK_TAIL(KP_, 64);                                                                                           \
  } while (0)
  if (KP == 16) TZK_TAIL_N(16);
  else if (KP == 32) TZK_TAIL_N(32);
  else TZK_TAIL_N(64);
#undef TZK_TAIL_N
#undef TZK_TAIL
#undef TZK_TAIL_ATTR
  if (cudaGetLastError() != cudaSuccess) return 3;
  const int len = out_len(K, N);
  TZK_LAUNCH((tower_tail_reduce_kernel), (len + 31) / 32, 256, 0, st, partial, grid, len, inv_m, out);
  return cudaGetLastError() == cudaSuccess ? 0 : 3;
}
}
```

torcheasyrec_b200/csrc/tzk_wgrad3x.cuh:

```cuda
#pragma once

constexpr int WG_THREADS = 256;
constexpr int WG_ROWS = 32;
constexpr int WG_BOX = WG_ROWS * 128;
constexpr int WG_A = 4 * WG_BOX, WG_B = 2 * WG_BOX;
constexpr int WG_STAGE = WG_A + WG_B;
constexpr int WG_STAGES = 4;
constexpr int WG_SRC = 3;

struct WgSources {
  int first[WG_SRC + 1];
  int col0[WG_SRC];
  int dst[WG_SRC];
  int width[WG_SRC];
};

struct WgParams {
  float* partial;
  int64_t M;
  int64_t slab_rows;
  int k_tiles;
  WgSources src;
};

__device__ __forceinline__ int wg_source(const WgSources& s, int box) {
  return box >= s.first[2] ? 2 : box >= s.first[1] ? 1 : 0;
}
__device__ __forceinline__ int wg_pick(const int* v, int s) { return s == 0 ? v[0] : s == 1 ? v[1] : v[2]; }

__global__ void __launch_bounds__(WG_THREADS, 2)
wgrad3x_kernel(const __grid_constant__ CUtensorMap map_x0, const __grid_constant__ CUtensorMap map_x1,
               const __grid_constant__ CUtensorMap map_x2, const __grid_constant__ CUtensorMap map_dz, WgParams p) {
  TZK_DYN_SMEM(uint8_t, smem);
  uint64_t* full = reinterpret_cast<uint64_t*>(smem + WG_STAGES * WG_STAGE);
  int* boxes = reinterpret_cast<int*>(full + WG_STAGES);

  const int warp = threadIdx.x >> 5, lane = threadIdx.x & 31, g = lane >> 2, t = lane & 3;
  const int jt = blockIdx.x % p.k_tiles;
  const int64_t slab = blockIdx.x / p.k_tiles;
  const int64_t row0 = slab * p.slab_rows;
  const int64_t rows = (p.M - row0 < p.slab_rows) ? p.M - row0 : p.slab_rows;
  const int num_c = (int)((rows + WG_ROWS - 1) / WG_ROWS);

  if (threadIdx.x == 0) {
    for (int s = 0; s < WG_STAGES; ++s) mbar_init(full + s, 1);
    fence_mbarrier_init();
    for (int b = 0; b < 4; ++b) {
      const int box = jt * 4 + b, s = wg_source(p.src, box);
      boxes[b] = s;
      boxes[4 + b] = wg_pick(p.src.col0, s) + 32 * (box - wg_pick(p.src.first, s));
    }
  }
  __syncthreads();
  auto load = [&](int c) {
    uint8_t* sb = smem + (c % WG_STAGES) * WG_STAGE;
    uint64_t* bar = full + c % WG_STAGES;
    const int r = (int)(row0 + (int64_t)c * WG_ROWS);
    mbar_expect_tx(bar, WG_A + WG_B);
#pragma unroll 1
    for (int b = 0; b < 4; ++b) {
      const int s = *reinterpret_cast<volatile int*>(boxes + b), col = *reinterpret_cast<volatile int*>(boxes + 4 + b);
      tma_load_2d(sb + b * WG_BOX, s == 0 ? &map_x0 : s == 1 ? &map_x1 : &map_x2, bar, col, r);
    }
#pragma unroll
    for (int b = 0; b < 2; ++b) tma_load_2d(sb + WG_A + b * WG_BOX, &map_dz, bar, b * 32, r);
  };
  if (threadIdx.x == 0)
    for (int c = 0; c < WG_STAGES && c < num_c; ++c) load(c);

  const int n0 = (warp & 3) * 16 + g;
  const int kc0 = (warp >> 2) * 64 + g;
  float acc[8][4], part[8][4];
#pragma unroll
  for (int nt = 0; nt < 8; ++nt)
#pragma unroll
    for (int q = 0; q < 4; ++q) acc[nt][q] = 0.f;
  for (int c = 0; c < num_c; ++c) {
    const int s = c % WG_STAGES;
    mbar_wait(full + s, (uint32_t)(c / WG_STAGES) & 1u);
    const float* xs = reinterpret_cast<const float*>(smem + s * WG_STAGE);
    const float* zs = reinterpret_cast<const float*>(smem + s * WG_STAGE + WG_A);
    auto at = [](const float* base, int m, int col) { return base[(col >> 5) * (WG_BOX / 4) + swz(m, col & 31)]; };
#pragma unroll
    for (int ks = 0; ks < WG_ROWS / 8; ++ks) {
#pragma unroll
      for (int nt = 0; nt < 8; ++nt)
#pragma unroll
        for (int q = 0; q < 4; ++q) part[nt][q] = 0.f;
      const int m = ks * 8 + t;
      const float a[4] = {at(zs, m, n0), at(zs, m, n0 + 8), at(zs, m + 4, n0), at(zs, m + 4, n0 + 8)};
      uint32_t ah[4], al[4];
#pragma unroll
      for (int i = 0; i < 4; ++i) {
        ah[i] = tf32_bits(a[i]);
        al[i] = tf32_bits(a[i] - __uint_as_float(ah[i]));
      }
#pragma unroll
      for (int nt = 0; nt < 8; ++nt) {
        const float b[2] = {at(xs, m, kc0 + 8 * nt), at(xs, m + 4, kc0 + 8 * nt)};
        uint32_t bh[2], bl[2];
#pragma unroll
        for (int i = 0; i < 2; ++i) {
          bh[i] = tf32_bits(b[i]);
          bl[i] = tf32_bits(b[i] - __uint_as_float(bh[i]));
        }
        mma_tf32(part[nt], al, bh);
        mma_tf32(part[nt], ah, bl);
        mma_tf32(part[nt], ah, bh);
      }
#pragma unroll
      for (int nt = 0; nt < 8; ++nt)
#pragma unroll
        for (int q = 0; q < 4; ++q) acc[nt][q] += part[nt][q];
    }
    __syncthreads();
    if (threadIdx.x == 0 && c + WG_STAGES < num_c) load(c + WG_STAGES);
  }
  float* out = p.partial + ((int64_t)slab * p.k_tiles + jt) * 128 * 64;
#pragma unroll
  for (int nt = 0; nt < 8; ++nt) {
    const int kcol = (warp >> 2) * 64 + nt * 8 + 2 * t;
#pragma unroll
    for (int q = 0; q < 4; ++q) out[(int64_t)(kcol + (q & 1)) * 64 + n0 + 8 * (q >> 1)] = acc[nt][q];
  }
}

__global__ void wgrad_reduce_kernel(const float* __restrict__ partial, int slabs, int k_pad, WgSources src,
                                    float* __restrict__ dw, int64_t ld_dw) {
  const int i = blockIdx.x * blockDim.x + threadIdx.x;
  if (i >= k_pad * 64) return;
  const int k = i >> 6, n = i & 63;
  const int s = wg_source(src, k >> 5);
  const int c = k - 32 * wg_pick(src.first, s);
  if (c >= wg_pick(src.width, s)) return;
  float acc = 0.f;
  for (int sl = 0; sl < slabs; ++sl) acc += partial[((int64_t)sl * k_pad + k) * 64 + n];
  dw[(int64_t)n * ld_dw + wg_pick(src.dst, s) + c] = acc;
}

template <auto Kernel = wgrad3x_kernel>
inline int wgrad3x_launch(const CUtensorMap (&mx)[WG_SRC], const CUtensorMap& mz, const WgSources& src, int64_t M,
                          int32_t slabs, float* partial, float* dw, int64_t ld_dw, cudaStream_t st,
                          size_t extra_smem = 0) {
  WgParams p;
  p.partial = partial;
  p.M = M;
  p.k_tiles = (src.first[WG_SRC] + 3) / 4;
  p.slab_rows = ((M + slabs - 1) / slabs + WG_ROWS - 1) / WG_ROWS * WG_ROWS;
  p.src = src;
  const int used = (int)((M + p.slab_rows - 1) / p.slab_rows);
  const size_t smem = (size_t)WG_STAGES * WG_STAGE + extra_smem + WG_STAGES * 8 + 8 * 4;
#ifndef TZK_CPU_SHIM
  static bool configured = false;
  if (!configured) {
    cudaFuncSetAttribute(Kernel, cudaFuncAttributeMaxDynamicSharedMemorySize, (int)smem);
    configured = true;
  }
#endif
  TZK_LAUNCH((Kernel), used * p.k_tiles, WG_THREADS, smem, st, mx[0], mx[1], mx[2], mz, p);
  TZK_LAUNCH((wgrad_reduce_kernel), (p.k_tiles * 128 * 64 + 255) / 256, 256, 0, st, partial, used, p.k_tiles * 128, src,
             dw, ld_dw);
  return cudaGetLastError() == cudaSuccess ? 0 : 3;
}
```

torcheasyrec_b200/dense_gemm.py:

```python

import ctypes
import os
from typing import Optional

import torch
from torch import nn

from .functional import autocast_dtype

_HERE = os.path.dirname(os.path.abspath(__file__))
_LIB_PATH = os.path.join(_HERE, "csrc", "libtzk_gemm.so")
_CUBLASLT_CANDIDATES = ["/usr/local/cuda/lib64/libcublasLt.so.12", "/usr/local/cuda-12.9/lib64/libcublasLt.so.12"]
_state = {"lib": None, "version": 0, "tried": False, "ws": {}, "emulated_calls": 0, "plain_calls": 0}


def _load():
    if _state["tried"]:
        return _state["lib"]
    _state["tried"] = True
    if os.environ.get("TZK_DENSE_GEMM", "") == "torch" or not os.path.exists(_LIB_PATH) or not torch.cuda.is_available():
        return None
    try:
        lib = ctypes.CDLL(_LIB_PATH)
        lib.tzg_init.restype = ctypes.c_long
# ... 171 lines not shown


def _g3_stream(t: torch.Tensor):
    return torch.cuda.current_stream().cuda_stream if t.is_cuda else None


def _g3_check(rc, what):
    if rc:
        raise RuntimeError(f"{what} failed with code {rc}")


def gemm3x(lib, x, w, bias, relu):
    M, K = x.shape
    N = w.shape[0]
    y = torch.empty((M, N), dtype=torch.float32, device=x.device)
    w_hi, w_lo = torch.empty_like(w), torch.empty_like(w)
    _g3_check(lib.tzk_gemm3x(x.data_ptr(), x.stride(0), w.data_ptr(), w.stride(0), None if bias is None else bias.data_ptr(),
                          M, N, K, int(relu), y.data_ptr(), N, w_hi.data_ptr(), w_lo.data_ptr(), _g3_stream(x)), "tzk_gemm3x")
    return y


def wgrad3x(lib, x, dz, slabs=SLABS):
    M, K = x.shape
    dw = torch.empty((64, K), dtype=torch.float32, device=x.device)
    part = torch.empty(lib.tzk_wgrad3x_partial_floats(K, slabs), dtype=torch.float32, device=x.device)
    _g3_check(lib.tzk_wgrad3x(x.data_ptr(), x.stride(0), dz.data_ptr(), dz.stride(0), M, K, slabs, part.data_ptr(),
                           dw.data_ptr(), K, _g3_stream(x)), "tzk_wgrad3x")
    return dw


class Gemm3xLinearFn(torch.autograd.Function):

    @staticmethod
    def forward(ctx, lib, x, weight, bias, relu, in_map):
        K, Kx = weight.shape[1], x.shape[1]
        w = weight.contiguous()
        if Kx != K:
            w = torch.zeros((weight.shape[0], Kx), dtype=weight.dtype, device=weight.device)
            for (src, dst, n) in (in_map or ((0, 0, K),)):
                w[:, dst:dst + n].copy_(weight[:, src:src + n])
        if not gemm3x_supported(x.shape[0], w.shape[0], Kx):
            raise ValueError(f"gemm3x covers N = 64 and input widths that are multiples of 112, got {tuple(w.shape)}")
        y = gemm3x(lib, x, w, bias, relu)
        ctx.lib, ctx.in_map, ctx.K = lib, in_map, K
        ctx.has_bias, ctx.relu = bias is not None, relu
        ctx.save_for_backward(x, w, y if relu else None)
        return y

    @staticmethod
    def backward(ctx, dy):
        x, w, y = ctx.saved_tensors
        lib = ctx.lib
        if dy.is_cuda and (ctx.has_bias or ctx.relu):
            from .kernels import default_kernels

            dz, colsum = default_kernels().act_bwd_colsum(dy.contiguous(), y, ctx.relu, want_dz=ctx.relu)
            dz = dz if ctx.relu else dy.contiguous()
            db = colsum if ctx.has_bias else None
        else:
            dz = (dy * (y > 0) if ctx.relu else dy).contiguous()
            db = dz.sum(0) if ctx.has_bias else None
        dx = dw = None
        if ctx.needs_input_grad[1]:
            dx = gemm3x(lib, dz, w.t().contiguous(), None, False)
        if ctx.needs_input_grad[2]:
            dw = wgrad3x(lib, x, dz)
            if w.shape[1] != ctx.K:
                segs = ctx.in_map or ((0, 0, ctx.K),)
                dw = torch.cat([dw[:, dst:dst + n] for (_, dst, n) in segs], dim=1) if len(segs) > 1 \
                    else dw[:, :ctx.K].contiguous()
        if not ctx.needs_input_grad[3]:
            db = None
        return None, dx, dw, db, None, None


class InteractWideFn(torch.autograd.Function):

    @staticmethod
    def forward(ctx, lib, dense, sparse, weight, bias, in_map):
        from .functional import _rows_contig
        from .kernels import default_kernels

        dense, sparse = _rows_contig(dense), _rows_contig(sparse)
        w = torch.zeros((weight.shape[0], 784), dtype=weight.dtype, device=weight.device)
        for (src, dst, n) in in_map:
            w[:, dst:dst + n].copy_(weight[:, src:src + n])
        y, pairs = default_kernels().interact_wide_fwd(dense, sparse, w, bias)
        ctx.in_map, ctx.has_bias = in_map, bias is not None
        ctx.save_for_backward(dense, sparse, pairs, w, y)
        return y

    @staticmethod
    def backward(ctx, dy):
        from .kernels import default_kernels

        dense, sparse, pairs, w, y = ctx.saved_tensors
        dz, colsum = default_kernels().act_bwd_colsum(dy.contiguous(), y, True, want_dz=True)
        d_dense = d_sparse = dw = None
        if ctx.needs_input_grad[1] or ctx.needs_input_grad[2]:
            d_dense, d_sparse = default_kernels().interact_wide_bwd(dz, w, dense, sparse)
        if ctx.needs_input_grad[3]:
            full = default_kernels().interact_wide_wgrad(dz, pairs, dense, sparse, SLABS)
            dw = torch.cat([full[:, dst:dst + n] for (_, dst, n) in ctx.in_map], dim=1)
        db = colsum if (ctx.has_bias and ctx.needs_input_grad[4]) else None
        return (None, d_dense if ctx.needs_input_grad[1] else None, d_sparse if ctx.needs_input_grad[2] else None, dw, db,
                None)


class InteractBf16Fn(torch.autograd.Function):

    IN_MAP = ((0, 0, 351), (351, 352, 432))

    @staticmethod
    def forward(ctx, dense, sparse):
        from .kernels import default_kernels

        ctx.save_for_backward(dense, sparse)
        return default_kernels().dot_interact27_fwd_bf16(dense, sparse)

    @staticmethod
    def backward(ctx, dx):
        from .kernels import default_kernels

        dense, sparse = ctx.saved_tensors
        if not (dx.stride(1) == 1 and dx.stride(0) % 8 == 0 and dx.data_ptr() % 16 == 0):
            dx = dx.contiguous()
        d_dense, d_sparse = default_kernels().dot_interact27_bwd_bf16(dx, dense, sparse)
        return (d_dense if ctx.needs_input_grad[0] else None), (d_sparse if ctx.needs_input_grad[1] else None)


def interact_bf16_usable(dense: Optional[torch.Tensor], sparse: torch.Tensor, num_sparse: int, dim: int) -> bool:
    return (dense is not None and sparse.is_cuda and autocast_dtype(sparse) == torch.bfloat16 and num_sparse == 26
            and dim == 16 and dense.dtype == torch.bfloat16 and sparse.dtype == torch.float32 and dense.dim() == 2
            and sparse.dim() == 2 and tuple(dense.shape[1:]) == (16,) and tuple(sparse.shape[1:]) == (416,)
            and dense.shape[0] == sparse.shape[0] >= 1
            and dense.stride(1) == 1 and dense.stride(0) % 4 == 0 and dense.data_ptr() % 8 == 0
            and sparse.stride(1) == 1 and sparse.stride(0) % 4 == 0 and sparse.data_ptr() % 16 == 0
            and os.environ.get("TZK_INTERACT_BF16", "1") != "0")


def interact_wide_usable(dense: Optional[torch.Tensor], sparse: torch.Tensor, weight: torch.Tensor,
                         num_sparse: int, dim: int) -> bool:
    return (dense is not None and autocast_dtype(sparse) is None and num_sparse == 26 and dim == 16 and dense.is_cuda and dense.dtype == torch.float32
            and sparse.dtype == torch.float32 and dense.dim() == 2 and tuple(dense.shape[1:]) == (16,)
            and sparse.dim() == 2 and tuple(sparse.shape[1:]) == (416,) and dense.shape[0] == sparse.shape[0] >= 256
            and all(t.stride(1) == 1 and t.stride(0) % 4 == 0 and t.data_ptr() % 16 == 0 for t in (dense, sparse))
            and weight.dtype == torch.float32 and tuple(weight.shape) == (64, 783)
            and os.environ.get("TZK_GEMM3X", "1") == "1" and os.environ.get("TZK_INTERACT_TC", "1") != "0"
            and os.environ.get("TZK_INTERACT_TC_FWD", "1") != "0" and os.environ.get("TZK_INTERACT_TC_BWD", "1") != "0"
            and not torch.backends.cuda.matmul.allow_tf32 and available() and _gemm3x_lib() is not None)


def _use_gemm3x(x: torch.Tensor, weight: torch.Tensor) -> bool:
    return (os.environ.get("TZK_GEMM3X", "1") == "1" and x.is_cuda and x.dim() == 2 and x.dtype == torch.float32
            and weight.dtype == torch.float32 and x.stride(1) == 1 and x.stride(0) % 4 == 0 and x.data_ptr() % 16 == 0
            and gemm3x_supported(x.shape[0], weight.shape[0], x.shape[1]) and _gemm3x_lib() is not None)


SMALL_MAX = 64


def _small(x: torch.Tensor, weight: torch.Tensor) -> bool:
    return (x.is_cuda and x.dim() == 2 and x.dtype == torch.float32 and weight.dtype == torch.float32
            and weight.shape[0] <= SMALL_MAX and weight.shape[1] <= SMALL_MAX and x.shape[1] == weight.shape[1]
            and x.shape[0] >= 1 and x.stride(1) == 1 and x.stride(0) >= x.shape[1]
            and os.environ.get("TZK_SMALL_LINEAR", "1") != "0")


class _BceFn(torch.autograd.Function):

    @staticmethod
    def forward(ctx, logits, labels):
        from .kernels import default_kernels

        loss, dz = default_kernels().bce_logits_fwd_bwd(logits.contiguous(), labels.contiguous())
        ctx.save_for_backward(dz)
        ctx.shape = logits.shape
        return loss

    @staticmethod
    def backward(ctx, g):
        (dz,) = ctx.saved_tensors
        return (dz * g).view(ctx.shape), None


class _TowerTailFn(torch.autograd.Function):

    @staticmethod
    def forward(ctx, y1, w1, b1, w2, b2, labels):
        from .kernels import default_kernels

        loss, logits, dy1, dw1, db1, dw2, db2 = default_kernels().tower_tail_bce(y1, w1, b1, w2, b2, labels)
        ctx.save_for_backward(dy1, dw1, db1, dw2, db2)
        ctx.has = (b1 is not None, b2 is not None)
        ctx.mark_non_differentiable(logits)
        return loss, logits

    @staticmethod
    def backward(ctx, g_loss, _g_logits):
        dy1, dw1, db1, dw2, db2 = ctx.saved_tensors
        return (dy1 * g_loss, dw1 * g_loss, (db1 * g_loss) if ctx.has[0] else None, dw2 * g_loss,
                (db2 * g_loss) if ctx.has[1] else None, None)


def tower_tail_usable(y1: torch.Tensor, w1: torch.Tensor, w2: torch.Tensor, labels: torch.Tensor) -> bool:
    return (autocast_dtype(y1) is None and y1.is_cuda and y1.dim() == 2 and y1.dtype == torch.float32 and w1.dtype == torch.float32
            and w1.shape[1] == y1.shape[1] <= 64 and w1.shape[0] <= 64 and tuple(w2.shape) == (1, w1.shape[0])
            and labels.dtype == torch.float32 and labels.numel() == y1.shape[0] >= 1 and y1.stride(1) == 1)


def tower_tail_bce(y1, w1, b1, w2, b2, labels):
    return _TowerTailFn.apply(y1, w1, b1, w2, b2, labels)


def bce_with_logits(logits: torch.Tensor, labels: torch.Tensor) -> torch.Tensor:
    if autocast_dtype(logits) is not None:
        logits, labels = logits.float(), labels.float()
    if (logits.is_cuda and logits.dtype == torch.float32 and labels.dtype == torch.float32 and logits.numel() >= 1
            and os.environ.get("TZK_SMALL_LINEAR", "1") != "0"):
        return _BceFn.apply(logits, labels)
    return torch.nn.functional.binary_cross_entropy_with_logits(logits, labels)


def _spread_weight(weight: torch.Tensor, width: int, in_map) -> torch.Tensor:
    N, K = weight.shape
    cols, c = [], 0
    for (src, dst, n) in (in_map or ((0, 0, K),)):
        if dst > c:
            cols.append(weight.new_zeros((N, dst - c)))
        cols.append(weight[:, src:src + n])
        c = dst + n
    if width > c:
        cols.append(weight.new_zeros((N, width - c)))
    return torch.cat(cols, dim=1)


def padded_width(n: int) -> int:
    return (n + 3) // 4 * 4


def _usable(x: torch.Tensor, weight: torch.Tensor) -> bool:
    return (x.is_cuda and x.dim() == 2 and x.dtype == torch.float32 and weight.dtype == torch.float32
            and x.shape[0] >= 256 and x.stride(1) == 1 and x.stride(0) >= x.shape[1]
            and not torch.backends.cuda.matmul.allow_tf32 and available())


def linear(x: torch.Tensor, weight: torch.Tensor, bias: Optional[torch.Tensor], relu: bool = False,
           in_map=None) -> torch.Tensor:
    K = weight.shape[1]
    if autocast_dtype(x) is not None:
        if x.dim() == 2 and (x.shape[1] != K or in_map is not None):
            if in_map is None and x.shape[1] != padded_width(K):
                raise RuntimeError(f"linear: input width {x.shape[1]} does not match in_features {K}")
            weight = _spread_weight(weight, x.shape[1], in_map)
        y = torch.nn.functional.linear(x, weight, bias)
        return torch.relu(y) if relu else y
    if in_map is None and _small(x, weight):
        return _SmallLinearFn.apply(x, weight, bias, relu)
    if x.dim() == 2 and (x.shape[1] != K or in_map is not None):
        if in_map is None and x.shape[1] != padded_width(K):
            raise RuntimeError(f"linear: input width {x.shape[1]} does not match in_features {K}")
        if not _usable(x, weight):
            x = x[:, :K] if in_map is None else torch.cat([x[:, d:d + n] for (_, d, n) in in_map], dim=1)
            in_map = None
    if _usable(x, weight):
        if _use_gemm3x(x, weight):
            return Gemm3xLinearFn.apply(_gemm3x_lib(), x, weight, bias, relu, in_map)
        return _LinearFn.apply(x, weight, bias, relu, in_map)
    y = torch.nn.functional.linear(x, weight, bias)
    return torch.relu(y) if relu else y


class Linear(nn.Linear):

    def forward(self, x: torch.Tensor) -> torch.Tensor:
        return linear(x, self.weight, self.bias)
```

torcheasyrec_b200/kernels.py:

```python

import ctypes
import math
import os
import threading
from dataclasses import dataclass
from typing import List, Optional, Sequence, Tuple

import torch

from ._lib import TzkError, check, lib

POOL_SUM, POOL_MEAN = 0, 1
OPT_SGD, OPT_ADAGRAD, OPT_ROWWISE_ADAGRAD, OPT_ADAM, OPT_PARTIAL_ROWWISE_ADAM = 0, 1, 2, 3, 4
OPT_LAMB, OPT_PARTIAL_ROWWISE_LAMB, OPT_LARS_SGD = 5, 6, 7
WD_NONE, WD_L2, WD_DECOUPLE = 0, 1, 2
LARS_ETA = 0.001
OPT_ACCUM_OUT = 100


@dataclass
class FeatureLayout:

    w_off: List[int]
    rows: List[int]
# ... 733 lines not shown
        return dx

    def dot_interact_fwd(self, dense: Optional[torch.Tensor], sparse: torch.Tensor, Ns: int, D: int,
                         copy_dense: bool, copy_sparse: bool, pad_to: int = 1, p_pad: int = 0) -> torch.Tensor:
        sparse, ld_s = _rows2d(sparse, "sparse")
        B = sparse.shape[0]
        ld_d = 0
        if dense is not None:
            dense, ld_d = _rows2d(dense, "dense")
        N = Ns + (dense is not None)
        width = N * (N - 1) // 2 + p_pad + (D if (copy_dense and dense is not None) else 0) + \
            (Ns * D if copy_sparse else 0)
        wp = (width + pad_to - 1) // pad_to * pad_to
        out = torch.empty((B, wp), dtype=torch.float32, device=sparse.device)
        if wp != width:
            out[:, width:].zero_()
        check(self._lib.tzk_dot_interact_fwd(_ptr(dense), ld_d, _ptr(sparse), ld_s, B, Ns, D, int(copy_dense),
                                             int(copy_sparse), p_pad, _ptr(out), wp, _stream()),
              "tzk_dot_interact_fwd")
        self.launches += 1
        return out

    def dot_interact_bwd(self, dense: Optional[torch.Tensor], sparse: torch.Tensor, d_out: torch.Tensor,
                         Ns: int, D: int, copy_dense: bool, copy_sparse: bool, p_pad: int = 0):
        sparse, ld_s = _rows2d(sparse, "sparse")
        d_out, ld_o = _rows2d(d_out, "d_out")
        B = sparse.shape[0]
        ld_d = 0
        d_dense = None
        if dense is not None:
            dense, ld_d = _rows2d(dense, "dense")
            d_dense = torch.empty((B, D), dtype=torch.float32, device=sparse.device)
        d_sparse = torch.empty((B, Ns * D), dtype=torch.float32, device=sparse.device)
        check(self._lib.tzk_dot_interact_bwd(_ptr(dense), ld_d, _ptr(sparse), ld_s, _ptr(d_out), ld_o, B, Ns, D,
                                             int(copy_dense), int(copy_sparse), p_pad, _ptr(d_dense), D,
                                             _ptr(d_sparse), Ns * D, _stream()), "tzk_dot_interact_bwd")
        self.launches += 1
        return d_dense, d_sparse

    def dot_interact27_fwd_bf16(self, dense: torch.Tensor, sparse: torch.Tensor) -> torch.Tensor:
        dense, ld_d = _rows2d_dtype(dense, torch.bfloat16, "dense")
        sparse, ld_s = _rows2d(sparse, "sparse")
        B = sparse.shape[0]
        if tuple(dense.shape) != (B, 16) or tuple(sparse.shape) != (B, 416):
            raise TzkError(f"dot_interact27_fwd_bf16: expected dense [B, 16] and sparse [B, 416], got "
                           f"{tuple(dense.shape)} and {tuple(sparse.shape)}")
        out = torch.empty((B, 784), dtype=torch.bfloat16, device=sparse.device)
        check(self._lib.tzk_dot_interact27_fwd_bf16(_ptr(dense), ld_d, _ptr(sparse), ld_s, B, _ptr(out), 784, _stream()),
              "tzk_dot_interact27_fwd_bf16")
        self.launches += 1
        return out

    def dot_interact27_bwd_bf16(self, d_out: torch.Tensor, dense: torch.Tensor, sparse: torch.Tensor):
        d_out, ld_o = _rows2d_dtype(d_out, torch.bfloat16, "d_out")
        dense, ld_d = _rows2d_dtype(dense, torch.bfloat16, "dense")
        sparse, ld_s = _rows2d(sparse, "sparse")
        B = sparse.shape[0]
        if tuple(d_out.shape) != (B, 784) or tuple(dense.shape) != (B, 16) or tuple(sparse.shape) != (B, 416):
            raise TzkError(f"dot_interact27_bwd_bf16: expected dX [B, 784], dense [B, 16] and sparse [B, 416], got "
                           f"{tuple(d_out.shape)}, {tuple(dense.shape)} and {tuple(sparse.shape)}")
        d_dense = torch.empty((B, 16), dtype=torch.bfloat16, device=sparse.device)
        d_sparse = torch.empty((B, 416), dtype=torch.float32, device=sparse.device)
        check(self._lib.tzk_dot_interact27_bwd_bf16(_ptr(d_out), ld_o, _ptr(dense), ld_d, _ptr(sparse), ld_s, B,
                                                    _ptr(d_dense), 16, _ptr(d_sparse), 416, _stream()),
              "tzk_dot_interact27_bwd_bf16")
        self.launches += 1
        return d_dense, d_sparse

    def interact_wide_fwd(self, dense: torch.Tensor, sparse: torch.Tensor, w: torch.Tensor, bias: Optional[torch.Tensor]):
        dense, ld_d = _rows2d(dense, "dense")
        sparse, ld_s = _rows2d(sparse, "sparse")
        w, ld_w = _rows2d(w, "w")
        B = dense.shape[0]
        y = torch.empty((B, 64), dtype=torch.float32, device=dense.device)
        pairs = torch.empty((B, 352), dtype=torch.float32, device=dense.device)
        ws = torch.empty((2, 64, 784), dtype=torch.float32, device=dense.device)
        check(self._lib.tzk_interact_wide_fwd(_ptr(dense), ld_d, _ptr(sparse), ld_s, _ptr(w), ld_w, _ptr(bias), B,
                                              _ptr(y), 64, _ptr(pairs), 352, _ptr(ws[0]), _ptr(ws[1]), _stream()),
              "tzk_interact_wide_fwd")
        self.launches += 2
        return y, pairs

    def interact_wide_wgrad(self, dz: torch.Tensor, pairs: torch.Tensor, dense: torch.Tensor, sparse: torch.Tensor,
                            slabs: int) -> torch.Tensor:
        dz, ld_z = _rows2d(dz, "dz")
        pairs, ld_p = _rows2d(pairs, "pairs")
        dense, ld_d = _rows2d(dense, "dense")
        sparse, ld_s = _rows2d(sparse, "sparse")
        B = dz.shape[0]
        dw = torch.empty((64, 784), dtype=torch.float32, device=dz.device)
        part = torch.empty(slabs * 896 * 64, dtype=torch.float32, device=dz.device)
        check(self._lib.tzk_interact_wide_wgrad(_ptr(dz), ld_z, _ptr(pairs), ld_p, _ptr(dense), ld_d, _ptr(sparse), ld_s,
                                                B, slabs, _ptr(part), _ptr(dw), 784, _stream()), "tzk_interact_wide_wgrad")
        self.launches += 2
        return dw

    def interact_wide_bwd(self, dz: torch.Tensor, w: torch.Tensor, dense: torch.Tensor, sparse: torch.Tensor):
        dz, ld_z = _rows2d(dz, "dz")
        w, ld_w = _rows2d(w, "w")
        dense, ld_d = _rows2d(dense, "dense")
        sparse, ld_s = _rows2d(sparse, "sparse")
        B = dz.shape[0]
        d_dense = torch.empty((B, 16), dtype=torch.float32, device=dz.device)
        d_sparse = torch.empty((B, 416), dtype=torch.float32, device=dz.device)
        wt = torch.empty((2, 784, 64), dtype=torch.float32, device=dz.device)
        check(self._lib.tzk_interact_wide_bwd(_ptr(dz), ld_z, _ptr(w), ld_w, _ptr(dense), ld_d, _ptr(sparse), ld_s, B,
                                              _ptr(d_dense), 16, _ptr(d_sparse), 416, _ptr(wt[0]), _ptr(wt[1]),
                                              _stream()), "tzk_interact_wide_bwd")
        self.launches += 2
        return d_dense, d_sparse

    def bias_act(self, y: torch.Tensor, bias: Optional[torch.Tensor], relu: bool) -> torch.Tensor:
        y, ld = _rows2d(y, "y")
        check(self._lib.tzk_bias_act(_ptr(y), ld, _ptr(bias), y.shape[0], y.shape[1], int(relu), _stream()),
              "tzk_bias_act")
        self.launches += 1
        return y

    def act_bwd_colsum(self, dy: torch.Tensor, y: Optional[torch.Tensor], relu: bool, want_dz: bool = True,
                       out: Optional[torch.Tensor] = None):
        dy, ld_dy = _rows2d(dy, "dy")
        M, N = dy.shape
        ld_y = 0
        if y is not None:
            y, ld_y = _rows2d(y, "y")
        if out is not None:
            dz, ld_dz = _rows2d(out, "out")
        else:
            dz, ld_dz = (torch.empty((M, N), dtype=torch.float32, device=dy.device) if want_dz else None), N
        colsum = torch.empty(N, dtype=torch.float32, device=dy.device)
        nb = self._lib.tzk_act_bwd_colsum_workspace_bytes(M, N)
        ws = self._workspace("colsum", nb, dy.device)
        check(self._lib.tzk_act_bwd_colsum(_ptr(dy), ld_dy, _ptr(y), ld_y, M, N, int(relu), _ptr(dz), ld_dz,
                                           _ptr(colsum), _ptr(ws), ws.numel(), _stream()), "tzk_act_bwd_colsum")
        self.launches += 2
        return dz, colsum
    def small_linear_fwd(self, x: torch.Tensor, w: torch.Tensor, bias: Optional[torch.Tensor],
                         relu: bool) -> torch.Tensor:
        x, ld_x = _rows2d(x, "x")
        _need(w, torch.float32, "w")
        M, K = x.shape
        N = w.shape[0]
        if w.shape[1] != K:
            raise TzkError(f"small_linear_fwd: x has {K} columns, w expects {w.shape[1]}")
        y = torch.empty((M, N), dtype=torch.float32, device=x.device)
        if M:
            check(self._lib.tzk_small_linear_fwd(_ptr(x), ld_x, _ptr(w), _ptr(bias), M, K, N, int(relu), _ptr(y), N,
                                                 _stream()), "tzk_small_linear_fwd")
            self.launches += 1
        return y

    def small_linear_bwd(self, x: torch.Tensor, w: torch.Tensor, y: Optional[torch.Tensor], dy: torch.Tensor,
                         relu: bool, want_dx: bool, want_db: bool):
        x, ld_x = _rows2d(x, "x")
        dy, ld_dy = _rows2d(dy, "dy")
        _need(w, torch.float32, "w")
        M, K = x.shape
        N = w.shape[0]
        ld_y = 0
        if relu:
            y, ld_y = _rows2d(y, "y")
        dx = torch.empty((M, K), dtype=torch.float32, device=x.device) if want_dx else None
        dw = torch.empty((N, K), dtype=torch.float32, device=x.device)
        db = torch.empty(N, dtype=torch.float32, device=x.device) if want_db else None
        nb = self._lib.tzk_small_linear_bwd_workspace_bytes(M, K, N)
        ws = self._workspace(("slb", K, N), nb, x.device)
        check(self._lib.tzk_small_linear_bwd(_ptr(x), ld_x, _ptr(w), _ptr(y) if relu else None, ld_y, _ptr(dy), ld_dy,
                                             M, K, N, int(relu), _ptr(dx), K, _ptr(dw), _ptr(db), _ptr(ws),
                                             ws.numel(), _stream()), "tzk_small_linear_bwd")
        self.launches += (2 + int(want_dx)) if _small_linear_rows_path(K, N) else 2
        return dx, dw, db

    def bce_logits_fwd_bwd(self, logits: torch.Tensor, labels: torch.Tensor, want_grad: bool = True):
        _need(logits, torch.float32, "logits")
        _need(labels, torch.float32, "labels")
        M = logits.numel()
        if labels.numel() != M:
            raise TzkError("bce_logits: logits and labels differ in size")
        loss = torch.empty((), dtype=torch.float32, device=logits.device)
        dz = torch.empty(M, dtype=torch.float32, device=logits.device) if want_grad else None
        nb = self._lib.tzk_bce_logits_workspace_bytes(M)
        ws = self._workspace("bce", nb, logits.device)
        check(self._lib.tzk_bce_logits_fwd_bwd(_ptr(logits), _ptr(labels), M, _ptr(loss), _ptr(dz), _ptr(ws),
                                               ws.numel(), _stream()), "tzk_bce_logits_fwd_bwd")
        self.launches += 2
        return loss, dz

    def tower_tail_bce(self, y1: torch.Tensor, w1: torch.Tensor, b1: Optional[torch.Tensor], w2: torch.Tensor,
                       b2: Optional[torch.Tensor], labels: torch.Tensor):
        y1, ld = _rows2d(y1, "y1")
        _need(w1, torch.float32, "w1")
        _need(w2, torch.float32, "w2")
        _need(labels, torch.float32, "labels")
        M, K = y1.shape
        N = w1.shape[0]
        if w1.shape != (N, K) or w2.numel() != N or labels.numel() != M:
            raise TzkError("tower_tail_bce: shapes do not chain")
        dev = y1.device
        logits = torch.empty(M, dtype=torch.float32, device=dev)
        dy1 = torch.empty((M, K), dtype=torch.float32, device=dev)
        out = torch.empty(N * K + 2 * N + 2, dtype=torch.float32, device=dev)
        nb = self._lib.tzk_tower_tail_bce_workspace_bytes(M, K, N)
        ws = self._workspace("tail", nb, dev)
        check(self._lib.tzk_tower_tail_bce(_ptr(y1), ld, _ptr(w1), _ptr(b1), _ptr(w2), _ptr(b2), _ptr(labels), M, K, N,
                                           _ptr(logits), _ptr(dy1), K, _ptr(out), _ptr(ws), ws.numel(), _stream()),
              "tzk_tower_tail_bce")
        self.launches += 2
        o = N * K
        return (out[o + 2 * N + 1], logits, dy1, out[:o].view(N, K), out[o:o + N], out[o + N:o + 2 * N].view(1, N),
                out[o + 2 * N:o + 2 * N + 1])

    def binned_auc_update(self, preds: torch.Tensor, labels: torch.Tensor, thresholds: torch.Tensor,
                          counts: torch.Tensor, invalid: torch.Tensor) -> None:
        if preds.dtype not in (torch.float32, torch.bfloat16):
            raise TzkError(f"binned_auc_update: predictions must be float32 or bfloat16, got {preds.dtype}")
        if labels.dtype not in (torch.float32, torch.int64):
            raise TzkError(f"binned_auc_update: labels must be float32 or int64, got {labels.dtype}")
        _need(preds, preds.dtype, "preds")
        _need(labels, labels.dtype, "labels")
        _need(thresholds, torch.float32, "thresholds")
        _need(counts, torch.int64, "counts")
        _need(invalid, torch.int64, "invalid")
        n, T = preds.numel(), thresholds.numel()
        if labels.numel() != n:
            raise TzkError(f"binned_auc_update: {n} predictions but {labels.numel()} labels")
        if T < 1 or counts.numel() != 2 * (T + 1) or invalid.numel() != 1:
            raise TzkError("binned_auc_update: counts must be [T + 1, 2] and invalid [1] for T >= 1 thresholds")
        check(self._lib.tzk_binned_auc_update(_ptr(preds), int(preds.dtype == torch.bfloat16), _ptr(labels),
                                              int(labels.dtype == torch.int64), n, _ptr(thresholds), T, _ptr(counts),
                                              _ptr(invalid), _stream()), "tzk_binned_auc_update")
        self.launches += int(n > 0)

    def _grid(self, work: int, per_sm: int, slices: int = 1) -> int:
        sms = getattr(self, "_sms", None)
        if sms is None:
            sms = self._sms = max(1, int(self._lib.tzk_sm_count()))
        return max(1, min(int(work), -(-per_sm * sms // slices)))

    def _batch_sums(self, key: str, grid: int, shapes, device):
        sizes = [math.prod(s) for s in shapes]
        partials = self._workspace(key, grid * sum(sizes) * 4, device)
        dparams = torch.empty(sum(sizes), dtype=torch.float32, device=device)
        return partials, dparams, [v.view(s) for v, s in zip(dparams.split(sizes), shapes)]

    def wukong_mix_fwd(self, x, w_fmb, gamma, beta, w_lcb, w_res, f: int):
        for t, nm in ((x, "x"), (w_fmb, "w_fmb"), (gamma, "gamma"), (beta, "beta"), (w_lcb, "w_lcb")):
            _need(t, torch.float32, nm)
        if w_res is not None:
            _need(w_res, torch.float32, "w_res")
        B, n, d = x.shape
        k, l = w_fmb.shape[1], w_lcb.shape[1]
        m = f + l
        ln_f = torch.empty((B, n * k), dtype=torch.float32, device=x.device)
        stats = torch.empty((B, 2), dtype=torch.float32, device=x.device)
        base = torch.empty((B, m, d), dtype=torch.float32, device=x.device)
        check(self._lib.tzk_wukong_mix_fwd(_ptr(x), _ptr(w_fmb), _ptr(gamma), _ptr(beta), _ptr(w_lcb), _ptr(w_res), B,
                                           n, d, k, f, l, self._grid(B, 8), _ptr(ln_f), _ptr(stats), _ptr(base),
                                           _stream()), "tzk_wukong_mix_fwd")
        self.launches += int(B > 0)
        return ln_f, stats, base

    def wukong_mix_bwd(self, x, w_fmb, gamma, w_lcb, w_res, f: int, stats, d_ln_f, d_base):
        for t, nm in ((x, "x"), (w_fmb, "w_fmb"), (gamma, "gamma"), (w_lcb, "w_lcb"), (stats, "stats"),
                      (d_ln_f, "d_ln_f"), (d_base, "d_base")):
            _need(t, torch.float32, nm)
        if w_res is not None:
            _need(w_res, torch.float32, "w_res")
        B, n, d = x.shape
        k, l = w_fmb.shape[1], w_lcb.shape[1]
        m = f + l
        grid = self._grid(B, 4)
        dx = torch.empty_like(x)
        partials, dparams, (dw_fmb, dw_lcb, dw_res, dgamma, dbeta) = self._batch_sums(
            "wukong_mix_bwd", grid, [(n, k), (n, l), (n, m if w_res is not None else 0), (n * k,), (n * k,)], x.device)
        check(self._lib.tzk_wukong_mix_bwd(_ptr(x), _ptr(w_fmb), _ptr(gamma), _ptr(w_lcb), _ptr(w_res), _ptr(stats),
                                           _ptr(d_ln_f), _ptr(d_base), B, n, d, k, f, l, grid, _ptr(dx),
                                           _ptr(partials), _ptr(dparams), _stream()), "tzk_wukong_mix_bwd")
        self.launches += 1 + int(B > 0)
        return dx, dw_fmb, dgamma, dbeta, dw_lcb, (dw_res if w_res is not None else None)

    def wukong_out_fwd(self, fmb_out, base, gamma, beta, f: int):
        for t, nm in ((fmb_out, "fmb_out"), (base, "base"), (gamma, "gamma"), (beta, "beta")):
            _need(t, torch.float32, nm)
        B, m, d = base.shape
        y = torch.empty_like(base)
        stats = torch.empty((B, m, 2), dtype=torch.float32, device=base.device)
        check(self._lib.tzk_wukong_out_fwd(_ptr(fmb_out), _ptr(base), _ptr(gamma), _ptr(beta), B, d, f, m - f,
                                           self._grid(-(-B * m // 128), 8), _ptr(y), _ptr(stats), _stream()),
              "tzk_wukong_out_fwd")
        self.launches += int(B > 0)
        return y, stats

    def wukong_out_bwd(self, fmb_out, base, gamma, f: int, stats, dy):
# ... 296 lines not shown
```

torcheasyrec_b200/rank_models.py:

```python

from typing import Any, Dict, List, Optional

import contextlib
import os
import struct

import torch
import torch.nn.functional as F
from torch import nn

from . import functional as Fn
from .dense_gemm import Linear as _Linear
from .batch import Batch
from .config import Message, config_to_kwargs
from .embedding_group import EmbeddingGroup
from .embedding_modules import SparseOptimizerSpec
from .features import BaseFeature
from .kernels import (OPT_ADAGRAD, OPT_ADAM, OPT_LAMB, OPT_LARS_SGD, OPT_PARTIAL_ROWWISE_ADAM, OPT_PARTIAL_ROWWISE_LAMB,
                      OPT_ROWWISE_ADAGRAD, OPT_SGD, WD_DECOUPLE, WD_L2, WD_NONE)


def _create_activation(act: str) -> Optional[nn.Module]:
    if not act:
        return None
# ... 284 lines not shown
        mods = self._metric_modules
        probs = "probs1" if self._ce_smoothing is not None else "probs"
        for metrics, loss_cfgs, label_name, suffix in self._updated_metric_heads():
            label = batch.labels[label_name]
            for mc in metrics:
                mods[mc.WhichOneof("metric") + suffix].update(predictions[probs + suffix], label)
            if losses is not None:
                for lc in loss_cfgs:
                    name = lc.WhichOneof("loss") + suffix
                    mods[name].update(losses[name], label.size(0))

    def compute_metric(self) -> Dict[str, torch.Tensor]:
        from .metrics import compute_all

        group, distributed = self._metric_sync
        return compute_all(self._metric_modules, group, distributed)

    def sparse_collections(self):
        return list(self.embedding_group.sparse_collections())

    def set_sparse_optimizer(self, spec: SparseOptimizerSpec) -> None:
        for coll in self.sparse_collections():
            coll.set_optimizer(spec)

    def dense_parameters(self):
        sparse_ids = {id(c.weights) for c in self.sparse_collections()}
        return [p for p in self.parameters() if id(p) not in sparse_ids and p.requires_grad]


class DLRM(RankModel):

    def __init__(self, model_config, features, labels, sample_weights=None, **kwargs) -> None:
        super().__init__(model_config, features, labels, sample_weights, **kwargs)
        self.init_input()
        eg = self.embedding_group
        self._sparse_group_name = eg.group_names()[0] if len(eg.group_names()) == 1 else "sparse"
        self.dense_mlp = None
        self._dense_group_name = "dense"
        if len(eg.group_names()) > 1 and eg.has_group(self._dense_group_name):
            self.dense_mlp = MLP(eg.group_total_dim(self._dense_group_name),
                                 **config_to_kwargs(self._model_config.dense_mlp))
        sparse_dims = eg.group_feature_dims(self._sparse_group_name)
        if len(set(sparse_dims.values())) > 1:
            raise Exception(f"sparse group feature dims must be the same, but we find {set(sparse_dims.values())}")
        self._per_sparse_dim = list(sparse_dims.values())[0]
        self._sparse_num = len(sparse_dims)
        sparse_dim = eg.group_total_dim(self._sparse_group_name)
        if self.dense_mlp and self._per_sparse_dim != self.dense_mlp.output_dim():
            raise Exception("dense mlp last hidden_unit must be the same sparse feature dim")
        self._feature_num = self._sparse_num + (1 if self.dense_mlp else 0)
        self.interaction = InteractionArch(self._feature_num)
        feature_dim = self.interaction.output_dim()
        if self.dense_mlp:
            feature_dim += self.dense_mlp.output_dim()
        if self._model_config.arch_with_sparse:
            feature_dim += sparse_dim
        self.final_mlp = MLP(feature_dim, **config_to_kwargs(self._model_config.final))
        self.output_mlp = _Linear(self.final_mlp.output_dim(), self._num_class)

    def predict(self, batch: Batch) -> Dict[str, torch.Tensor]:
        dense_in = self._dense_group_input(batch) if self.dense_mlp else None
        side = None
        if dense_in is not None and dense_in.is_cuda:
            from .kernels import _unvalidated_switch

            if _unvalidated_switch("TZK_DLRM_BOTTOM_STREAM"):
                side = getattr(self, "_bottom_stream", None)
                if side is None:
                    side = self._bottom_stream = torch.cuda.Stream(device=dense_in.device)
        if side is not None:
            cur = torch.cuda.current_stream()
            side.wait_stream(cur)
            with torch.cuda.stream(side):
                dense_feat = self.dense_mlp(dense_in)
        else:
            dense_feat = self.dense_mlp(dense_in) if dense_in is not None else None
        grouped = self.build_input(batch)
        if side is not None:
            cur.wait_stream(side)
            dense_feat.record_stream(cur)
        sparse = grouped[self._sparse_group_name]
        if self.dense_mlp and dense_feat is None:
            dense_feat = self.dense_mlp(grouped[self._dense_group_name])
        x = self._interact_wide(dense_feat, sparse)
        if x is not None:
            in_map, start = None, 1
        elif self._interact_bf16_ok(dense_feat, sparse):
            from .dense_gemm import InteractBf16Fn

            x, in_map, start = InteractBf16Fn.apply(dense_feat, sparse), InteractBf16Fn.IN_MAP, 0
        else:
            x, in_map = Fn.dlrm_interaction(dense_feat, sparse, self._sparse_num, self._per_sparse_dim,
                                            with_dense=True,
                                            with_sparse=bool(self._model_config.arch_with_sparse), aligned=True)
            start = 0
        fused = self._fused_tail(batch, x, in_map, start)
        if fused is not None:
            return fused
        for i, layer in enumerate(list(self.final_mlp.mlp)[start:], start):
            x = layer(x, in_map) if (i == 0 and in_map is not None) else layer(x)
        return self._output_to_prediction(self.output_mlp(x))

    def _interact_wide(self, dense_feat: Optional[torch.Tensor], sparse: torch.Tensor) -> Optional[torch.Tensor]:
        from .dense_gemm import InteractWideFn, _gemm3x_lib, interact_wide_usable

        first = self.final_mlp.mlp[0].perceptron
        if not (self._model_config.arch_with_sparse and len(first) == 2 and isinstance(first[1], nn.ReLU)
                and interact_wide_usable(dense_feat, sparse, first[0].weight, self._sparse_num, self._per_sparse_dim)):
            return None
        in_map = ((0, 0, 351), (351, 352, 432))
        return InteractWideFn.apply(_gemm3x_lib(), dense_feat, sparse, first[0].weight, first[0].bias, in_map)

    def _interact_bf16_ok(self, dense_feat: Optional[torch.Tensor], sparse: torch.Tensor) -> bool:
        from .dense_gemm import interact_bf16_usable

        return bool(self._model_config.arch_with_sparse) and interact_bf16_usable(dense_feat, sparse, self._sparse_num,
                                                                                   self._per_sparse_dim)

    def _fused_tail(self, batch: Batch, all_feat: torch.Tensor, in_map, start: int = 0):
        from .dense_gemm import tower_tail_bce, tower_tail_usable

        self._tail_loss = None
        layers = list(self.final_mlp.mlp)
        if (not self.training or Fn.autocast_dtype(all_feat) is not None or not torch.is_grad_enabled() or not all_feat.is_cuda or self._num_class != 1
                or not layers or self._label_name not in batch.labels or os.environ.get("TZK_FUSED_TAIL", "1") == "0"):
            return None
        last = layers[-1].perceptron
        if not (len(last) == 2 and isinstance(last[1], nn.ReLU)):
            return None
        label = batch.labels[self._label_name].to(torch.float32)
        w1, b1 = last[0].weight, last[0].bias
        w2, b2 = self.output_mlp.weight, self.output_mlp.bias
        if start >= len(layers):
            return None
        x = all_feat
        for i, layer in enumerate(layers[start:-1], start):
            x = layer(x, in_map) if (i == 0 and in_map is not None) else layer(x)
        if len(layers) == 1 and in_map is not None:
            return None
        if not tower_tail_usable(x, w1, w2, label):
            return None
        loss, logits = tower_tail_bce(x, w1, b1, w2, b2, label)
        self._tail_loss = loss
        return {"logits": logits, "probs": torch.sigmoid(logits)}


    def _dense_group_input(self, batch: Batch) -> Optional[torch.Tensor]:
        eg = self.embedding_group
        impl = next(iter(eg.emb_impls.values())) if len(eg.emb_impls) == 1 else None
        if impl is None or not impl.has_dense:
            return None
        key = next(iter(eg.emb_impls.keys()))
        kt = batch.dense_features.get(key)
        names = impl._group_to_shared_feature_names.get(self._dense_group_name)
        if kt is None or names is None or list(kt.keys()) != list(names):
            return None
        return kt.values()


class DeepFM(RankModel):

    def __init__(self, model_config, features, labels, sample_weights=None, **kwargs) -> None:
        super().__init__(model_config, features, labels, sample_weights, **kwargs)
        self.init_input()
        eg = self.embedding_group
        self.fm = FactorizationMachine()
        fm_group = "fm" if eg.has_group("fm") else "deep"
        self._fm_feature_dims = eg.group_dims(fm_group)
        if len(set(self._fm_feature_dims)) > 1:
            raise ValueError(f"fm feature dims must be the same, but got {self._fm_feature_dims}")
        self.deep_mlp = MLP(in_features=eg.group_total_dim("deep"), **config_to_kwargs(self._model_config.deep))
        final_dim = self.deep_mlp.output_dim()
        if self._model_config.HasField("final"):
            self.final_mlp = MLP(in_features=1 + self._fm_feature_dims[0] + final_dim,
                                 **config_to_kwargs(self._model_config.final))
            final_dim = self.final_mlp.output_dim()
        self.output_mlp = _Linear(final_dim, self._num_class)

    def predict(self, batch: Batch) -> Dict[str, torch.Tensor]:
        grouped = self.build_input(batch)
        y_wide = torch.sum(grouped["wide"], dim=1, keepdim=True)
        deep_feat = grouped["deep"]
        y_deep = self.deep_mlp(deep_feat)
        fm_feat = grouped["fm"] if self.embedding_group.has_group("fm") else deep_feat
        y_fm = self.fm(fm_feat.reshape(-1, len(self._fm_feature_dims), self._fm_feature_dims[0]))
        if self._model_config.HasField("final"):
            y = self.output_mlp(self.final_mlp(torch.cat([y_wide, y_fm, y_deep], dim=1)))
        else:
            y = y_wide + torch.sum(y_fm, dim=1, keepdim=True) + self.output_mlp(y_deep)
        return self._output_to_prediction(y)


class MultiTowerDIN(RankModel):

    def __init__(self, model_config, features, labels, sample_weights=None, **kwargs) -> None:
        super().__init__(model_config, features, labels, sample_weights, **kwargs)
        self.init_input()
        eg = self.embedding_group
        self.towers = nn.ModuleDict()
        total = 0
        for tower in self._model_config.towers:
            self.towers[tower.input] = MLP(eg.group_total_dim(tower.input), **config_to_kwargs(tower.mlp))
            total += self.towers[tower.input].output_dim()
        self.din_towers = nn.ModuleList()
        for tower in (self._model_config.din_towers if self._model_type == "multi_tower_din" else []):
            g = tower.input
            enc = DINEncoder(eg.group_total_dim(f"{g}.sequence"), eg.group_total_dim(f"{g}.query"), g,
                             attn_mlp=config_to_kwargs(tower.attn_mlp))
            self.din_towers.append(enc)
            total += enc.output_dim()
        if len(self.din_towers) and os.environ.get("TZK_DIN_JAGGED", "1") != "0":
            eg.set_jagged_for_attention([t.input for t in self._model_config.din_towers])
        final_dim = total
        if self._model_config.HasField("final"):
            self.final_mlp = MLP(in_features=total, **config_to_kwargs(self._model_config.final))
            final_dim = self.final_mlp.output_dim()
        self.output_mlp = _Linear(final_dim, self._num_class)

    def predict(self, batch: Batch) -> Dict[str, torch.Tensor]:
        grouped = self.build_input(batch)
        outs = [mlp(grouped[k]) for k, mlp in self.towers.items()]
        outs += [din(grouped) for din in self.din_towers]
        x = torch.cat(outs, dim=-1)
        if self._model_config.HasField("final"):
            x = self.final_mlp(x)
        return self._output_to_prediction(self.output_mlp(x))


# ... 917 lines not shown
```

Measured before the change: 52.67 million.

## Fuse interact-wide layer with tower tail BCE and fold loss scale into backward

Adds a combined autograd path for DLRM when the final MLP has two layers: the wide interaction layer feeds directly into the fused tower-tail BCE kernel. The tail kernel now applies the ReLU mask itself and emits the column sum for the first layer's bias gradient. The interact-wide backward and wgrad kernels take an optional device-side gradient scale, so a separate scaling pass over dz is not needed. This removes intermediate elementwise kernels and launches, at the cost of extra shared memory in the tail kernel and more dispatch conditions.

```diff
diff --git a/include/tzk.h b/include/tzk.h
--- a/include/tzk.h
+++ b/include/tzk.h
@@ -159,12 +159,20 @@
                           int64_t ld_dense, const float* sparse, int64_t ld_sparse, int64_t M, float* d_dense,
                           int64_t ld_ddense, float* d_sparse, int64_t ld_dsparse, float* wt_hi, float* wt_lo,
                           tzk_stream_t stream);
+int tzk_interact_wide_bwd_scaled(const float* dz, int64_t ld_dz, const float* dz_scale, const float* w, int64_t ld_w,
+                                 const float* dense, int64_t ld_dense, const float* sparse, int64_t ld_sparse, int64_t M,
+                                 float* d_dense, int64_t ld_ddense, float* d_sparse, int64_t ld_dsparse, float* wt_hi,
+                                 float* wt_lo, tzk_stream_t stream);
 int tzk_interact_wide_fwd(const float* dense, int64_t ld_dense, const float* sparse, int64_t ld_sparse, const float* w,
                           int64_t ld_w, const float* bias, int64_t M, float* y, int64_t ld_y, float* pairs,
                           int64_t ld_pairs, float* w_hi, float* w_lo, tzk_stream_t stream);
 int tzk_interact_wide_wgrad(const float* dz, int64_t ld_dz, const float* pairs, int64_t ld_pairs, const float* dense,
                             int64_t ld_dense, const float* sparse, int64_t ld_sparse, int64_t M, int32_t slabs,
                             float* partial, float* dw, int64_t ld_dw, tzk_stream_t stream);
+int tzk_interact_wide_wgrad_scaled(const float* dz, int64_t ld_dz, const float* dz_scale, const float* pairs,
+                                   int64_t ld_pairs, const float* dense, int64_t ld_dense, const float* sparse,
+                                   int64_t ld_sparse, int64_t M, int32_t slabs, float* partial, float* dw,
+                                   int64_t ld_dw, tzk_stream_t stream);
 
 int tzk_bias_act(float* y, int64_t ld_y, const float* bias, int64_t M, int32_t N, int32_t relu,
                  tzk_stream_t stream);
@@ -185,7 +193,7 @@
 size_t tzk_tower_tail_bce_workspace_bytes(int64_t M, int32_t K, int32_t N);
 int tzk_tower_tail_bce(const float* y1, int64_t ld_y, const float* w1, const float* b1, const float* w2, const float* b2,
                        const float* labels, int64_t M, int32_t K, int32_t N, float* logits, float* dy1, int64_t ld_dy,
-                       float* out, void* workspace, size_t workspace_bytes, tzk_stream_t stream);
+                       float* colsum, float* out, void* workspace, size_t workspace_bytes, tzk_stream_t stream);
 int tzk_bce_logits_fwd_bwd(const float* logits, const float* labels, int64_t M, float* loss, float* dlogits,
                            void* workspace, size_t workspace_bytes, tzk_stream_t stream);
 
diff --git a/torcheasyrec_b200/_lib.py b/torcheasyrec_b200/_lib.py
--- a/torcheasyrec_b200/_lib.py
+++ b/torcheasyrec_b200/_lib.py
@@ -152,12 +152,17 @@
     ),
     "tzk_interact_wide_bwd": (
         c_int32, [P, c_int64, P, c_int64, P, c_int64, P, c_int64, c_int64, P, c_int64, P, c_int64, P, P, P]),
+    "tzk_interact_wide_bwd_scaled": (
+        c_int32, [P, c_int64, P, P, c_int64, P, c_int64, P, c_int64, c_int64, P, c_int64, P, c_int64, P, P, P]),
     "tzk_interact_wide_fwd": (
         c_int32, [P, c_int64, P, c_int64, P, c_int64, P, c_int64, P, c_int64, P, c_int64, P, P, P]),
     "tzk_interact_wide_wgrad": (
         c_int32, [P, c_int64, P, c_int64, P, c_int64, P, c_int64, c_int64, c_int32, P, P, c_int64, P]),
+    "tzk_interact_wide_wgrad_scaled": (
+        c_int32, [P, c_int64, P, P, c_int64, P, c_int64, P, c_int64, c_int64, c_int32, P, P, c_int64, P]),
     "tzk_tower_tail_bce_workspace_bytes": (c_size_t, [c_int64, c_int32, c_int32]),
-    "tzk_tower_tail_bce": (c_int32, [P, c_int64, P, P, P, P, P, c_int64, c_int32, c_int32, P, P, c_int64, P, P, c_size_t, P]),
+    "tzk_tower_tail_bce": (
+        c_int32, [P, c_int64, P, P, P, P, P, c_int64, c_int32, c_int32, P, P, c_int64, P, P, P, c_size_t, P]),
     "tzk_din_attn_input_fwd": (c_int32, [P, c_int64, c_int32, P, P, c_int32, c_int32, c_int64, P, P]),
     "tzk_din_attn_input_bwd": (c_int32, [P, P, c_int64, c_int32, P, P, c_int32, c_int32, c_int64, P, P, P]),
     "tzk_jagged_softmax_wsum_fwd": (c_int32, [P, P, P, c_int32, c_int32, c_int32, c_int64, P, P, P]),
diff --git a/torcheasyrec_b200/csrc/tzk_common.cuh b/torcheasyrec_b200/csrc/tzk_common.cuh
--- a/torcheasyrec_b200/csrc/tzk_common.cuh
+++ b/torcheasyrec_b200/csrc/tzk_common.cuh
@@ -10,6 +10,7 @@
 namespace tzk {
 
 void set_error(const char* fmt, ...);
+void colsum_final(const float* partial, int64_t n_blocks, int N, float* colsum, cudaStream_t st);
 
 inline cudaStream_t as_stream(tzk_stream_t s) { return reinterpret_cast<cudaStream_t>(s); }
 
diff --git a/torcheasyrec_b200/csrc/tzk_dense.cu b/torcheasyrec_b200/csrc/tzk_dense.cu
--- a/torcheasyrec_b200/csrc/tzk_dense.cu
+++ b/torcheasyrec_b200/csrc/tzk_dense.cu
@@ -763,6 +763,10 @@
 }
 }
 
+void tzk::colsum_final(const float* partial, int64_t n_blocks, int N, float* colsum, cudaStream_t st) {
+  colsum_final_kernel<<<(N + 31) / 32, 256, 0, st>>>(partial, n_blocks, N, colsum);
+}
+
 extern "C" int tzk_bias_act(float* y, int64_t ld_y, const float* bias, int64_t M, int32_t N, int32_t relu,
                             tzk_stream_t stream) {
   TZK_REQUIRE(M >= 0 && N >= 1, "bias_act: bad sizes");
@@ -797,7 +801,7 @@
   act_bwd_colsum_kernel<<<(unsigned)nb, kThreads, 0, as_stream(stream)>>>(dy, ld_dy, y, ld_y, M, N, relu, dz, ld_dz,
                                                                           partial);
   TZK_CHECK_LAUNCH("act_bwd_colsum_kernel");
-  colsum_final_kernel<<<(N + 31) / 32, 256, 0, as_stream(stream)>>>(partial, nb, N, colsum);
+  colsum_final(partial, nb, N, colsum, as_stream(stream));
   TZK_CHECK_LAUNCH("colsum_final_kernel");
   return 0;
 }
diff --git a/torcheasyrec_b200/csrc/tzk_interact_wide.cu b/torcheasyrec_b200/csrc/tzk_interact_wide.cu
--- a/torcheasyrec_b200/csrc/tzk_interact_wide.cu
+++ b/torcheasyrec_b200/csrc/tzk_interact_wide.cu
@@ -77,6 +77,7 @@
   float* d_dense; int64_t ld_ddense;
   float* d_sparse; int64_t ld_dsparse;
   int64_t M;
+  const float* dz_scale;
 };
 
 __global__ void __launch_bounds__(FB_THREADS, 1)
@@ -129,6 +130,7 @@
     FB_STAMP(tile, 0);
     float a[8][4];
     {
+      const float zk = p.dz_scale ? __ldg(p.dz_scale) : 1.f;
       const int s = (int)(item0 % FB_STAGES);
       mbar_wait(full + 2 * s, (uint32_t)(item0 / FB_STAGES) & 1u);
       mbar_wait(full + 2 * s + 1, (uint32_t)(item0 / FB_STAGES) & 1u);
@@ -137,10 +139,10 @@
       for (int kk = 0; kk < 8; ++kk) {
         const float* box = zs + (kk >> 2) * (FB_HALF / 4);
         const int k0 = (kk & 3) * 8 + t, k1 = k0 + 4;
-        a[kk][0] = box[swz(r, k0)];
-        a[kk][1] = box[swz(r + 8, k0)];
-        a[kk][2] = box[swz(r, k1)];
-        a[kk][3] = box[swz(r + 8, k1)];
+        a[kk][0] = box[swz(r, k0)] * zk;
+        a[kk][1] = box[swz(r + 8, k0)] * zk;
+        a[kk][2] = box[swz(r, k1)] * zk;
+        a[kk][3] = box[swz(r + 8, k1)] * zk;
       }
     }
     __syncthreads();
@@ -437,13 +439,14 @@
     const float* xs = reinterpret_cast<const float*>(smem + s * WG_STAGE);
     const float* zs = reinterpret_cast<const float*>(smem + s * WG_STAGE + WG_A);
     auto at = [](const float* base, int m, int col) { return base[(col >> 5) * (WG_BOX / 4) + swz(m, col & 31)]; };
+    const float zk = p.dz_scale ? __ldg(p.dz_scale) : 1.f;
 #pragma unroll
     for (int h = 0; h < 2; ++h) {
       const int m = 4 * tq + 16 * h;
       float hi[4], lo[4];
 #pragma unroll
       for (int j = 0; j < 4; ++j) {
-        const float v = at(zs, m + j, tn);
+        const float v = at(zs, m + j, tn) * zk;
         hi[j] = tf32_rna(v);
         lo[j] = tf32_rna(v - hi[j]);
       }
@@ -506,10 +509,11 @@
 }
 #endif
 
-extern "C" int tzk_interact_wide_bwd(const float* dz, int64_t ld_dz, const float* w, int64_t ld_w, const float* dense,
-                                     int64_t ld_dense, const float* sparse, int64_t ld_sparse, int64_t M, float* d_dense,
-                                     int64_t ld_ddense, float* d_sparse, int64_t ld_dsparse, float* wt_hi, float* wt_lo,
-                                     tzk_stream_t stream) {
+extern "C" int tzk_interact_wide_bwd_scaled(const float* dz, int64_t ld_dz, const float* dz_scale, const float* w,
+                                            int64_t ld_w, const float* dense, int64_t ld_dense, const float* sparse,
+                                            int64_t ld_sparse, int64_t M, float* d_dense, int64_t ld_ddense,
+                                            float* d_sparse, int64_t ld_dsparse, float* wt_hi, float* wt_lo,
+                                            tzk_stream_t stream) {
   TZK_REQUIRE(M > 0, "interact_wide_bwd: M must be positive");
   TZK_REQUIRE(ld_w >= tzk_itc::kRow, "interact_wide_bwd: w needs %d columns", tzk_itc::kRow);
   const int64_t lds[] = {ld_dz, ld_w, ld_dense, ld_sparse, ld_ddense, ld_dsparse};
@@ -532,6 +536,7 @@
   FbParams p;
   p.dense = dense; p.ld_dense = ld_dense; p.sparse = sparse; p.ld_sparse = ld_sparse;
   p.d_dense = d_dense; p.ld_ddense = ld_ddense; p.d_sparse = d_sparse; p.ld_dsparse = ld_dsparse; p.M = M;
+  p.dz_scale = dz_scale;
 #ifndef TZK_CPU_SHIM
   static bool configured = false;
   if (!configured) {
@@ -543,6 +548,14 @@
   TZK_LAUNCH((interact_wide_bwd_kernel), (unsigned)(tiles < sms ? tiles : sms), FB_THREADS, FB_SMEM, st, mz, mh, ml, p);
   TZK_CHECK_LAUNCH("interact_wide_bwd_kernel");
   return 0;
+}
+
+extern "C" int tzk_interact_wide_bwd(const float* dz, int64_t ld_dz, const float* w, int64_t ld_w, const float* dense,
+                                     int64_t ld_dense, const float* sparse, int64_t ld_sparse, int64_t M, float* d_dense,
+                                     int64_t ld_ddense, float* d_sparse, int64_t ld_dsparse, float* wt_hi, float* wt_lo,
+                                     tzk_stream_t stream) {
+  return tzk_interact_wide_bwd_scaled(dz, ld_dz, nullptr, w, ld_w, dense, ld_dense, sparse, ld_sparse, M, d_dense,
+                                      ld_ddense, d_sparse, ld_dsparse, wt_hi, wt_lo, stream);
 }
 
 extern "C" int tzk_interact_wide_fwd(const float* dense, int64_t ld_dense, const float* sparse, int64_t ld_sparse,
@@ -579,10 +592,10 @@
   return 0;
 }
 
-extern "C" int tzk_interact_wide_wgrad(const float* dz, int64_t ld_dz, const float* pairs, int64_t ld_pairs,
-                                       const float* dense, int64_t ld_dense, const float* sparse, int64_t ld_sparse,
-                                       int64_t M, int32_t slabs, float* partial, float* dw, int64_t ld_dw,
-                                       tzk_stream_t stream) {
+extern "C" int tzk_interact_wide_wgrad_scaled(const float* dz, int64_t ld_dz, const float* dz_scale,
+                                              const float* pairs, int64_t ld_pairs, const float* dense, int64_t ld_dense,
+                                              const float* sparse, int64_t ld_sparse, int64_t M, int32_t slabs,
+                                              float* partial, float* dw, int64_t ld_dw, tzk_stream_t stream) {
   TZK_REQUIRE(M > 0 && slabs > 0, "interact_wide_wgrad: M and slabs must be positive");
   TZK_REQUIRE(ld_dw >= tzk_itc::kRow, "interact_wide_wgrad: dw needs %d columns", tzk_itc::kRow);
   const int64_t lds[] = {ld_dz, ld_pairs, ld_dense, ld_sparse};
@@ -598,7 +611,16 @@
   const WgSources src = {{0, FB_PAIR_CHUNKS, FB_CHUNKS - 1, FB_CHUNKS}, {0, 0, 0}, {0, FF_SPARSE0, tzk_itc::kInter},
                          {tzk_itc::kInter, tzk_itc::kRow - FF_SPARSE0, tzk_itc::kD}};
   TZK_REQUIRE(wgrad3x_launch<interact_wide_wgrad_kernel>(mx, mz, src, M, slabs, partial, dw, ld_dw,
-                                                         reinterpret_cast<cudaStream_t>(stream), 2 * WW_ZT) == 0,
+                                                         reinterpret_cast<cudaStream_t>(stream), 2 * WW_ZT,
+                                                         dz_scale) == 0,
               "interact_wide_wgrad: launch failed");
   return 0;
 }
+
+extern "C" int tzk_interact_wide_wgrad(const float* dz, int64_t ld_dz, const float* pairs, int64_t ld_pairs,
+                                       const float* dense, int64_t ld_dense, const float* sparse, int64_t ld_sparse,
+                                       int64_t M, int32_t slabs, float* partial, float* dw, int64_t ld_dw,
+                                       tzk_stream_t stream) {
+  return tzk_interact_wide_wgrad_scaled(dz, ld_dz, nullptr, pairs, ld_pairs, dense, ld_dense, sparse, ld_sparse, M,
+                                        slabs, partial, dw, ld_dw, stream);
+}
diff --git a/torcheasyrec_b200/csrc/tzk_tower.cu b/torcheasyrec_b200/csrc/tzk_tower.cu
--- a/torcheasyrec_b200/csrc/tzk_tower.cu
+++ b/torcheasyrec_b200/csrc/tzk_tower.cu
@@ -440,8 +440,8 @@
 
 extern "C" int tzk_tower_tail_bce(const float* y1, int64_t ld_y, const float* w1, const float* b1, const float* w2,
                                   const float* b2, const float* labels, int64_t M, int32_t K, int32_t N, float* logits,
-                                  float* dy1, int64_t ld_dy, float* out, void* workspace, size_t workspace_bytes,
-                                  tzk_stream_t stream) {
+                                  float* dy1, int64_t ld_dy, float* colsum, float* out, void* workspace,
+                                  size_t workspace_bytes, tzk_stream_t stream) {
   TZK_REQUIRE(M >= 1, "tower_tail_bce: empty batch");
   TZK_REQUIRE(tzk_tail::supported(K, N), "tower_tail_bce: K=%d, N=%d must be in [1, 64]", K, N);
   TZK_REQUIRE(y1 && w1 && w2 && labels && logits && dy1 && out, "tower_tail_bce: NULL argument");
@@ -449,7 +449,12 @@
   TZK_REQUIRE(workspace && workspace_bytes >= tzk_tower_tail_bce_workspace_bytes(M, K, N),
               "tower_tail_bce: workspace too small");
   const int rc = tzk_tail::run(y1, ld_y, w1, b1, w2, b2, labels, M, K, N, logits, dy1, ld_dy, out, workspace,
-                               workspace_bytes, as_stream(stream));
+                               workspace_bytes, as_stream(stream), colsum != nullptr);
   TZK_REQUIRE(rc == 0, "tower_tail_bce: tzk_tail::run failed with code %d", rc);
+  if (colsum) {
+    colsum_final(static_cast<const float*>(workspace) + tzk_tail::colsum_offset(M, K, N), tzk_tail::tiles(M), K, colsum,
+                 as_stream(stream));
+    TZK_CHECK_LAUNCH("colsum_final_kernel");
+  }
   return 0;
 }
diff --git a/torcheasyrec_b200/csrc/tzk_tower_tail.cuh b/torcheasyrec_b200/csrc/tzk_tower_tail.cuh
--- a/torcheasyrec_b200/csrc/tzk_tower_tail.cuh
+++ b/torcheasyrec_b200/csrc/tzk_tower_tail.cuh
@@ -12,17 +12,23 @@
   const int64_t t = (M + kRows - 1) / kRows;
   return (int)(t < 1 ? 1 : (t < kMaxCtas ? t : kMaxCtas));
 }
-inline size_t workspace_bytes(int64_t M, int K, int N) { return (size_t)grid_for(M) * out_len(K, N) * sizeof(float); }
-inline size_t smem_bytes(int KP, int NP) {
-  return ((size_t)NP * KP + 2 * NP + (size_t)kRows * (KP + 4) + 2 * (size_t)kRows * NP + 2 * kRows) * sizeof(float);
-}
-
-template <int KP, int NP>
+inline int64_t tiles(int64_t M) { return (M + kRows - 1) / kRows; }
+inline size_t colsum_offset(int64_t M, int K, int N) { return (size_t)grid_for(M) * out_len(K, N); }
+inline size_t workspace_bytes(int64_t M, int K, int N) {
+  return (colsum_offset(M, K, N) + (size_t)tiles(M) * K) * sizeof(float);
+}
+inline size_t smem_bytes(int KP, int NP, bool mask) {
+  return ((size_t)NP * KP + 2 * NP + (size_t)(mask ? 2 : 1) * kRows * (KP + 4) + 2 * (size_t)kRows * NP + 2 * kRows) *
+         sizeof(float);
+}
+
+template <int KP, int NP, bool kMask>
 __global__ void __launch_bounds__(kRows)
 tower_tail_bce_kernel(const float* __restrict__ y1, int64_t ld_y, const float* __restrict__ w1,
                       const float* __restrict__ b1, const float* __restrict__ w2, const float* __restrict__ b2,
                       const float* __restrict__ labels, int64_t M, int K, int N, float inv_m, int rows_per_cta,
-                      float* __restrict__ logits, float* __restrict__ dy1, int64_t ld_dy, float* __restrict__ partial) {
+                      float* __restrict__ logits, float* __restrict__ dy1, int64_t ld_dy, float* __restrict__ partial,
+                      float* __restrict__ zsum) {
   constexpr int R = kRows, KC = KP / 4, NC = NP / 4, XS = KP + 4;
   constexpr int NB = (KC * NC + R - 1) / R;
   TZK_DYN_SMEM(float, sm);
@@ -34,6 +40,7 @@
   float* Hg = Dh + R * NP;
   float* Dz = Hg + R * NP;
   float* Ls = Dz + R;
+  float* Zs = Ls + R;
   const int tid = threadIdx.x;
   for (int i = tid; i < NP * KP; i += R) {
     const int n = i / KP, k = i - n * KP;
@@ -125,6 +132,14 @@
         a.z = fmaf(h[n], w4.z, a.z);
         a.w = fmaf(h[n], w4.w, a.w);
       }
+      if constexpr (kMask) {
+        const float4 y4 = *reinterpret_cast<const float4*>(xr + 4 * c);
+        a.x = y4.x > 0.f ? a.x : 0.f;
+        a.y = y4.y > 0.f ? a.y : 0.f;
+        a.z = y4.z > 0.f ? a.z : 0.f;
+        a.w = y4.w > 0.f ? a.w : 0.f;
+        *reinterpret_cast<float4*>(Zs + tid * XS + 4 * c) = a;
+      }
       if (live && 4 * c < K) {
         float* p = dy1 + row * ld_dy + 4 * c;
         if (vout) {
@@ -167,6 +182,20 @@
       for (int r = 0; r < R; ++r) {
         accz += Dz[r];
         accl += Ls[r];
+      }
+    }
+    if constexpr (kMask) {
+      const int c = tid - (R - KP);
+      if (c >= 0 && c < K) {
+        float s[4] = {0.f, 0.f, 0.f, 0.f};
+#pragma unroll 4
+        for (int r = 0; r < R; r += 4)
+#pragma unroll
+          for (int j = 0; j < 4; ++j) s[j] += Zs[(r + j) * XS + c];
+        float v = 0.f;
+#pragma unroll
+        for (int j = 0; j < 4; ++j) v += s[j];
+        zsum[t0 / R * K + c] = v;
       }
     }
     __syncthreads();
@@ -216,7 +245,7 @@
 
 inline int run(const float* y1, int64_t ld_y, const float* w1, const float* b1, const float* w2, const float* b2,
                const float* labels, int64_t M, int32_t K, int32_t N, float* logits, float* dy1, int64_t ld_dy,
-               float* out, void* workspace, size_t workspace_bytes_, cudaStream_t st) {
+               float* out, void* workspace, size_t workspace_bytes_, cudaStream_t st, bool mask = false) {
   if (M < 1 || !supported(K, N) || !y1 || !w1 || !w2 || !labels || !logits || !dy1 || !out || ld_y < K || ld_dy < K) return 1;
   if (workspace_bytes_ < workspace_bytes(M, K, N)) return 2;
   const int KP = K <= 16 ? 16 : (K <= 32 ? 32 : 64);
@@ -225,30 +254,37 @@
   int rows_per_cta = (int)((M + grid - 1) / grid);
   rows_per_cta = (rows_per_cta + kRows - 1) / kRows * kRows;
   const float inv_m = 1.0f / (float)M;
-  const size_t smem = smem_bytes(KP, NP);
+  const size_t smem = smem_bytes(KP, NP, mask);
   float* partial = static_cast<float*>(workspace);
+  float* zsum = partial + colsum_offset(M, K, N);
 #ifdef TZK_CPU_SHIM
-#define TZK_TAIL_ATTR(KP_, NP_)
+#define TZK_TAIL_ATTR(KP_, NP_, MASK_)
 #else
-#define TZK_TAIL_ATTR(KP_, NP_)                                                                                       \
+#define TZK_TAIL_ATTR(KP_, NP_, MASK_)                                                                                \
   if (smem > 48 * 1024)                                                                                               \
-    cudaFuncSetAttribute(tower_tail_bce_kernel<KP_, NP_>, cudaFuncAttributeMaxDynamicSharedMemorySize, (int)smem);
+    cudaFuncSetAttribute(tower_tail_bce_kernel<KP_, NP_, MASK_>, cudaFuncAttributeMaxDynamicSharedMemorySize, (int)smem);
 #endif
-#define TZK_TAIL(KP_, NP_)                                                                                            \
+#define TZK_TAIL(KP_, NP_, MASK_)                                                                                     \
   do {                                                                                                                \
-    TZK_TAIL_ATTR(KP_, NP_)                                                                                           \
-    TZK_LAUNCH((tower_tail_bce_kernel<KP_, NP_>), grid, kRows, smem, st, y1, ld_y, w1, b1, w2, b2, labels, M, K, N,   \
-               inv_m, rows_per_cta, logits, dy1, ld_dy, partial);                                                     \
+    TZK_TAIL_ATTR(KP_, NP_, MASK_)                                                                                    \
+    TZK_LAUNCH((tower_tail_bce_kernel<KP_, NP_, MASK_>), grid, kRows, smem, st, y1, ld_y, w1, b1, w2, b2, labels, M,  \
+               K, N, inv_m, rows_per_cta, logits, dy1, ld_dy, partial, zsum);                                         \
   } while (0)
-#define TZK_TAIL_N(KP_)                                                                                               \
+#define TZK_TAIL_N(KP_, MASK_)                                                                                        \
   do {                                                                                                                \
-    if (NP == 16) TZK_TAIL(KP_, 16);                                                                                  \
-    else if (NP == 32) TZK_TAIL(KP_, 32);                                                                             \
-    else TZK_TAIL(KP_, 64);                                                                                           \
+    if (NP == 16) TZK_TAIL(KP_, 16, MASK_);                                                                           \
+    else if (NP == 32) TZK_TAIL(KP_, 32, MASK_);                                                                      \
+    else TZK_TAIL(KP_, 64, MASK_);                                                                                    \
   } while (0)
-  if (KP == 16) TZK_TAIL_N(16);
-  else if (KP == 32) TZK_TAIL_N(32);
-  else TZK_TAIL_N(64);
+#define TZK_TAIL_K(MASK_)                                                                                             \
+  do {                                                                                                                \
+    if (KP == 16) TZK_TAIL_N(16, MASK_);                                                                              \
+    else if (KP == 32) TZK_TAIL_N(32, MASK_);                                                                         \
+    else TZK_TAIL_N(64, MASK_);                                                                                       \
+  } while (0)
+  if (mask) TZK_TAIL_K(true);
+  else TZK_TAIL_K(false);
+#undef TZK_TAIL_K
 #undef TZK_TAIL_N
 #undef TZK_TAIL
 #undef TZK_TAIL_ATTR
diff --git a/torcheasyrec_b200/csrc/tzk_wgrad3x.cuh b/torcheasyrec_b200/csrc/tzk_wgrad3x.cuh
--- a/torcheasyrec_b200/csrc/tzk_wgrad3x.cuh
+++ b/torcheasyrec_b200/csrc/tzk_wgrad3x.cuh
@@ -21,6 +21,7 @@
   int64_t slab_rows;
   int k_tiles;
   WgSources src;
+  const float* dz_scale;
 };
 
 __device__ __forceinline__ int wg_source(const WgSources& s, int box) {
@@ -141,9 +142,10 @@
 template <auto Kernel = wgrad3x_kernel>
 inline int wgrad3x_launch(const CUtensorMap (&mx)[WG_SRC], const CUtensorMap& mz, const WgSources& src, int64_t M,
                           int32_t slabs, float* partial, float* dw, int64_t ld_dw, cudaStream_t st,
-                          size_t extra_smem = 0) {
+                          size_t extra_smem = 0, const float* dz_scale = nullptr) {
   WgParams p;
   p.partial = partial;
+  p.dz_scale = dz_scale;
   p.M = M;
   p.k_tiles = (src.first[WG_SRC] + 3) / 4;
   p.slab_rows = ((M + slabs - 1) / slabs + WG_ROWS - 1) / WG_ROWS * WG_ROWS;
diff --git a/torcheasyrec_b200/dense_gemm.py b/torcheasyrec_b200/dense_gemm.py
--- a/torcheasyrec_b200/dense_gemm.py
+++ b/torcheasyrec_b200/dense_gemm.py
@@ -277,9 +277,7 @@
         from .kernels import default_kernels
 
         dense, sparse = _rows_contig(dense), _rows_contig(sparse)
-        w = torch.zeros((weight.shape[0], 784), dtype=weight.dtype, device=weight.device)
-        for (src, dst, n) in in_map:
-            w[:, dst:dst + n].copy_(weight[:, src:src + n])
+        w = _interact_wide_weight(weight, in_map)
         y, pairs = default_kernels().interact_wide_fwd(dense, sparse, w, bias)
         ctx.in_map, ctx.has_bias = in_map, bias is not None
         ctx.save_for_backward(dense, sparse, pairs, w, y)
@@ -302,6 +300,49 @@
                 None)
 
 
+def _interact_wide_weight(weight: torch.Tensor, in_map) -> torch.Tensor:
+    w = torch.zeros((weight.shape[0], 784), dtype=weight.dtype, device=weight.device)
+    for (src, dst, n) in in_map:
+        w[:, dst:dst + n].copy_(weight[:, src:src + n])
+    return w
+
+
+class InteractWideTailFn(torch.autograd.Function):
+
+    @staticmethod
+    def forward(ctx, dense, sparse, weight, bias, in_map, w1, b1, w2, b2, labels):
+        from .functional import _rows_contig
+        from .kernels import default_kernels
+
+        K = default_kernels()
+        dense, sparse = _rows_contig(dense), _rows_contig(sparse)
+        w = _interact_wide_weight(weight, in_map)
+        y1, pairs = K.interact_wide_fwd(dense, sparse, w, bias)
+        loss, logits, dz, dw1, db1, dw2, db2, colsum = K.tower_tail_bce(y1, w1, b1, w2, b2, labels, relu_dz=True)
+        ctx.save_for_backward(dense, sparse, pairs, w, dz, colsum, dw1, db1, dw2, db2)
+        ctx.in_map, ctx.has = in_map, (bias is not None, b1 is not None, b2 is not None)
+        ctx.mark_non_differentiable(logits)
+        return loss, logits
+
+    @staticmethod
+    def backward(ctx, g_loss, _g_logits):
+        from .kernels import default_kernels
+
+        K = default_kernels()
+        dense, sparse, pairs, w, dz, colsum, dw1, db1, dw2, db2 = ctx.saved_tensors
+        g = g_loss.reshape(1)
+        need = ctx.needs_input_grad
+        d_dense = d_sparse = dw = None
+        if need[0] or need[1]:
+            d_dense, d_sparse = K.interact_wide_bwd(dz, w, dense, sparse, scale=g)
+        if need[2]:
+            full = K.interact_wide_wgrad(dz, pairs, dense, sparse, SLABS, scale=g)
+            dw = torch.cat([full[:, dst:dst + n] for (_, dst, n) in ctx.in_map], dim=1)
+        return (d_dense if need[0] else None, d_sparse if need[1] else None, dw,
+                (colsum * g_loss) if (ctx.has[0] and need[3]) else None, None, dw1 * g_loss,
+                (db1 * g_loss) if ctx.has[1] else None, dw2 * g_loss, (db2 * g_loss) if ctx.has[2] else None, None)
+
+
 class InteractBf16Fn(torch.autograd.Function):
 
     IN_MAP = ((0, 0, 351), (351, 352, 432))
@@ -385,7 +426,7 @@
     def forward(ctx, y1, w1, b1, w2, b2, labels):
         from .kernels import default_kernels
 
-        loss, logits, dy1, dw1, db1, dw2, db2 = default_kernels().tower_tail_bce(y1, w1, b1, w2, b2, labels)
+        loss, logits, dy1, dw1, db1, dw2, db2, _ = default_kernels().tower_tail_bce(y1, w1, b1, w2, b2, labels)
         ctx.save_for_backward(dy1, dw1, db1, dw2, db2)
         ctx.has = (b1 is not None, b2 is not None)
         ctx.mark_non_differentiable(logits)
@@ -399,9 +440,17 @@
 
 
 def tower_tail_usable(y1: torch.Tensor, w1: torch.Tensor, w2: torch.Tensor, labels: torch.Tensor) -> bool:
-    return (autocast_dtype(y1) is None and y1.is_cuda and y1.dim() == 2 and y1.dtype == torch.float32 and w1.dtype == torch.float32
-            and w1.shape[1] == y1.shape[1] <= 64 and w1.shape[0] <= 64 and tuple(w2.shape) == (1, w1.shape[0])
-            and labels.dtype == torch.float32 and labels.numel() == y1.shape[0] >= 1 and y1.stride(1) == 1)
+    return (autocast_dtype(y1) is None and y1.is_cuda and y1.dim() == 2 and y1.dtype == torch.float32
+            and y1.stride(1) == 1 and _tail_layers_usable(y1.shape[0], y1.shape[1], w1, w2, labels))
+
+
+def _tail_layers_usable(M: int, K: int, w1: torch.Tensor, w2: torch.Tensor, labels: torch.Tensor) -> bool:
+    return (w1.dtype == torch.float32 and w1.shape[1] == K <= 64 and w1.shape[0] <= 64
+            and tuple(w2.shape) == (1, w1.shape[0]) and labels.dtype == torch.float32 and labels.numel() == M >= 1)
+
+
+def interact_wide_tail_usable(sparse: torch.Tensor, w1: torch.Tensor, w2: torch.Tensor, labels: torch.Tensor) -> bool:
+    return _tail_layers_usable(sparse.shape[0], 64, w1, w2, labels)
 
 
 def tower_tail_bce(y1, w1, b1, w2, b2, labels):
diff --git a/torcheasyrec_b200/kernels.py b/torcheasyrec_b200/kernels.py
--- a/torcheasyrec_b200/kernels.py
+++ b/torcheasyrec_b200/kernels.py
@@ -839,7 +839,7 @@
         return y, pairs
 
     def interact_wide_wgrad(self, dz: torch.Tensor, pairs: torch.Tensor, dense: torch.Tensor, sparse: torch.Tensor,
-                            slabs: int) -> torch.Tensor:
+                            slabs: int, scale: Optional[torch.Tensor] = None) -> torch.Tensor:
         dz, ld_z = _rows2d(dz, "dz")
         pairs, ld_p = _rows2d(pairs, "pairs")
         dense, ld_d = _rows2d(dense, "dense")
@@ -847,12 +847,16 @@
         B = dz.shape[0]
         dw = torch.empty((64, 784), dtype=torch.float32, device=dz.device)
         part = torch.empty(slabs * 896 * 64, dtype=torch.float32, device=dz.device)
-        check(self._lib.tzk_interact_wide_wgrad(_ptr(dz), ld_z, _ptr(pairs), ld_p, _ptr(dense), ld_d, _ptr(sparse), ld_s,
-                                                B, slabs, _ptr(part), _ptr(dw), 784, _stream()), "tzk_interact_wide_wgrad")
+        if scale is not None and _need(scale, torch.float32, "scale").numel() != 1:
+            raise TzkError("scale: expected one element")
+        check(self._lib.tzk_interact_wide_wgrad_scaled(_ptr(dz), ld_z, _ptr(scale), _ptr(pairs), ld_p, _ptr(dense), ld_d,
+                                                       _ptr(sparse), ld_s, B, slabs, _ptr(part), _ptr(dw), 784,
+                                                       _stream()), "tzk_interact_wide_wgrad_scaled")
         self.launches += 2
         return dw
 
-    def interact_wide_bwd(self, dz: torch.Tensor, w: torch.Tensor, dense: torch.Tensor, sparse: torch.Tensor):
+    def interact_wide_bwd(self, dz: torch.Tensor, w: torch.Tensor, dense: torch.Tensor, sparse: torch.Tensor,
+                          scale: Optional[torch.Tensor] = None):
         dz, ld_z = _rows2d(dz, "dz")
         w, ld_w = _rows2d(w, "w")
         dense, ld_d = _rows2d(dense, "dense")
@@ -861,9 +865,12 @@
         d_dense = torch.empty((B, 16), dtype=torch.float32, device=dz.device)
         d_sparse = torch.empty((B, 416), dtype=torch.float32, device=dz.device)
         wt = torch.empty((2, 784, 64), dtype=torch.float32, device=dz.device)
-        check(self._lib.tzk_interact_wide_bwd(_ptr(dz), ld_z, _ptr(w), ld_w, _ptr(dense), ld_d, _ptr(sparse), ld_s, B,
-                                              _ptr(d_dense), 16, _ptr(d_sparse), 416, _ptr(wt[0]), _ptr(wt[1]),
-                                              _stream()), "tzk_interact_wide_bwd")
+        if scale is not None and _need(scale, torch.float32, "scale").numel() != 1:
+            raise TzkError("scale: expected one element")
+        check(self._lib.tzk_interact_wide_bwd_scaled(_ptr(dz), ld_z, _ptr(scale), _ptr(w), ld_w, _ptr(dense), ld_d,
+                                                     _ptr(sparse), ld_s, B, _ptr(d_dense), 16, _ptr(d_sparse), 416,
+                                                     _ptr(wt[0]), _ptr(wt[1]), _stream()),
+              "tzk_interact_wide_bwd_scaled")
         self.launches += 2
         return d_dense, d_sparse
 
@@ -944,7 +951,7 @@
         return loss, dz
 
     def tower_tail_bce(self, y1: torch.Tensor, w1: torch.Tensor, b1: Optional[torch.Tensor], w2: torch.Tensor,
-                       b2: Optional[torch.Tensor], labels: torch.Tensor):
+                       b2: Optional[torch.Tensor], labels: torch.Tensor, relu_dz: bool = False):
         y1, ld = _rows2d(y1, "y1")
         _need(w1, torch.float32, "w1")
         _need(w2, torch.float32, "w2")
@@ -957,15 +964,16 @@
         logits = torch.empty(M, dtype=torch.float32, device=dev)
         dy1 = torch.empty((M, K), dtype=torch.float32, device=dev)
         out = torch.empty(N * K + 2 * N + 2, dtype=torch.float32, device=dev)
+        colsum = torch.empty(K, dtype=torch.float32, device=dev) if relu_dz else None
         nb = self._lib.tzk_tower_tail_bce_workspace_bytes(M, K, N)
         ws = self._workspace("tail", nb, dev)
         check(self._lib.tzk_tower_tail_bce(_ptr(y1), ld, _ptr(w1), _ptr(b1), _ptr(w2), _ptr(b2), _ptr(labels), M, K, N,
-                                           _ptr(logits), _ptr(dy1), K, _ptr(out), _ptr(ws), ws.numel(), _stream()),
-              "tzk_tower_tail_bce")
-        self.launches += 2
+                                           _ptr(logits), _ptr(dy1), K, _ptr(colsum), _ptr(out), _ptr(ws), ws.numel(),
+                                           _stream()), "tzk_tower_tail_bce")
+        self.launches += 3 if relu_dz else 2
         o = N * K
         return (out[o + 2 * N + 1], logits, dy1, out[:o].view(N, K), out[o:o + N], out[o + N:o + 2 * N].view(1, N),
-                out[o + 2 * N:o + 2 * N + 1])
+                out[o + 2 * N:o + 2 * N + 1], colsum)
 
     def binned_auc_update(self, preds: torch.Tensor, labels: torch.Tensor, thresholds: torch.Tensor,
                           counts: torch.Tensor, invalid: torch.Tensor) -> None:
diff --git a/torcheasyrec_b200/rank_models.py b/torcheasyrec_b200/rank_models.py
--- a/torcheasyrec_b200/rank_models.py
+++ b/torcheasyrec_b200/rank_models.py
@@ -390,6 +390,9 @@
         sparse = grouped[self._sparse_group_name]
         if self.dense_mlp and dense_feat is None:
             dense_feat = self.dense_mlp(grouped[self._dense_group_name])
+        fused = self._interact_wide_tail(batch, dense_feat, sparse)
+        if fused is not None:
+            return fused
         x = self._interact_wide(dense_feat, sparse)
         if x is not None:
             in_map, start = None, 1
@@ -410,14 +413,34 @@
         return self._output_to_prediction(self.output_mlp(x))
 
     def _interact_wide(self, dense_feat: Optional[torch.Tensor], sparse: torch.Tensor) -> Optional[torch.Tensor]:
-        from .dense_gemm import InteractWideFn, _gemm3x_lib, interact_wide_usable
-
+        from .dense_gemm import InteractWideFn, _gemm3x_lib
+
+        if not self._interact_wide_ok(dense_feat, sparse):
+            return None
         first = self.final_mlp.mlp[0].perceptron
-        if not (self._model_config.arch_with_sparse and len(first) == 2 and isinstance(first[1], nn.ReLU)
-                and interact_wide_usable(dense_feat, sparse, first[0].weight, self._sparse_num, self._per_sparse_dim)):
+        return InteractWideFn.apply(_gemm3x_lib(), dense_feat, sparse, first[0].weight, first[0].bias, self._WIDE_IN_MAP)
+
+    _WIDE_IN_MAP = ((0, 0, 351), (351, 352, 432))
+
+    def _interact_wide_ok(self, dense_feat: Optional[torch.Tensor], sparse: torch.Tensor) -> bool:
+        from .dense_gemm import interact_wide_usable
+
+        first = self.final_mlp.mlp[0].perceptron
+        return bool(self._model_config.arch_with_sparse and len(first) == 2 and isinstance(first[1], nn.ReLU)
+                    and interact_wide_usable(dense_feat, sparse, first[0].weight, self._sparse_num, self._per_sparse_dim))
+
+    def _interact_wide_tail(self, batch: Batch, dense_feat: Optional[torch.Tensor], sparse: torch.Tensor):
+        from .dense_gemm import InteractWideTailFn, interact_wide_tail_usable
+
+        if len(self.final_mlp.mlp) != 2 or not self._interact_wide_ok(dense_feat, sparse):
             return None
-        in_map = ((0, 0, 351), (351, 352, 432))
-        return InteractWideFn.apply(_gemm3x_lib(), dense_feat, sparse, first[0].weight, first[0].bias, in_map)
+        tail = self._tail_inputs(batch, sparse)
+        if tail is None or not interact_wide_tail_usable(sparse, tail[0], tail[2], tail[4]):
+            return None
+        first = self.final_mlp.mlp[0].perceptron[0]
+        loss, logits = InteractWideTailFn.apply(dense_feat, sparse, first.weight, first.bias, self._WIDE_IN_MAP, *tail)
+        self._tail_loss = loss
+        return {"logits": logits, "probs": torch.sigmoid(logits)}
 
     def _interact_bf16_ok(self, dense_feat: Optional[torch.Tensor], sparse: torch.Tensor) -> bool:
         from .dense_gemm import interact_bf16_usable
@@ -430,15 +453,10 @@
 
         self._tail_loss = None
         layers = list(self.final_mlp.mlp)
-        if (not self.training or Fn.autocast_dtype(all_feat) is not None or not torch.is_grad_enabled() or not all_feat.is_cuda or self._num_class != 1
-                or not layers or self._label_name not in batch.labels or os.environ.get("TZK_FUSED_TAIL", "1") == "0"):
+        tail = self._tail_inputs(batch, all_feat)
+        if tail is None:
             return None
-        last = layers[-1].perceptron
-        if not (len(last) == 2 and isinstance(last[1], nn.ReLU)):
-            return None
-        label = batch.labels[self._label_name].to(torch.float32)
-        w1, b1 = last[0].weight, last[0].bias
-        w2, b2 = self.output_mlp.weight, self.output_mlp.bias
+        w1, b1, w2, b2, label = tail
         if start >= len(layers):
             return None
         x = all_feat
@@ -452,6 +470,17 @@
         self._tail_loss = loss
         return {"logits": logits, "probs": torch.sigmoid(logits)}
 
+
+    def _tail_inputs(self, batch: Batch, feat: torch.Tensor):
+        layers = list(self.final_mlp.mlp)
+        if (not self.training or Fn.autocast_dtype(feat) is not None or not torch.is_grad_enabled() or not feat.is_cuda or self._num_class != 1
+                or not layers or self._label_name not in batch.labels or os.environ.get("TZK_FUSED_TAIL", "1") == "0"):
+            return None
+        last = layers[-1].perceptron
+        if not (len(last) == 2 and isinstance(last[1], nn.ReLU)):
+            return None
+        return (last[0].weight, last[0].bias, self.output_mlp.weight, self.output_mlp.bias,
+                batch.labels[self._label_name].to(torch.float32))
 
     def _dense_group_input(self, batch: Batch) -> Optional[torch.Tensor]:
         eg = self.embedding_group
```

After: 54.88 million (median of 6 runs). 1.04x the previous value.
